# jkflying/opencalibration

Hardware: AMD Instinct MI355X
Metric: images/sec end-to-end (extract+match+relax) on synthetic aerial grid; LM iters/sec (higher is better)
Workload: dtype f32 (extract) + fp4 0/1 bits, f32 accumulate, exact (match) + f64 (RANSAC, relax)

## Files before the change

include/oc_host.h:

```cpp
#ifndef OC_HOST_H
#define OC_HOST_H

#include <stddef.h>
#include <stdint.h>

#include "ochip.h"

#ifdef __cplusplus
extern "C"
{
#endif

    size_t och_subsample(const double *loc, const float *strength, size_t n, double spacing, size_t count,
                         uint64_t *out);

    size_t och_matches_from_device(const ochip_match *raw, const uint64_t *idx1, size_t n1, const uint64_t *idx2,
                                   size_t n2, uint64_t *out_i1, uint64_t *out_i2, double *out_dist);

    typedef struct och_graph och_graph;
    och_graph *och_graph_create(void);
    void och_graph_destroy(och_graph *g);
    const char *och_last_error(const och_graph *g);
    uint32_t och_graph_add_model(och_graph *g, const double *m10);
    uint64_t och_graph_add_image(och_graph *g, const double *loc, const float *strength, const uint64_t *desc, size_t n,
                                 size_t num_sparse, uint32_t model, const double *position3);
    uint64_t och_graph_add_edge(och_graph *g, uint64_t source_id, uint64_t dest_id, const double *H9, int is_homography,
                                size_t n_inliers, const double *inl_px4, const uint64_t *inl_idx3, size_t n_matches,
                                const uint64_t *match_idx2, const double *match_dist, const double *poses32);
    void och_graph_get_orientations(const och_graph *g, double *ori );
    void och_link_match_work(const och_graph *g, double *out3);
    size_t och_graph_num_nodes(const och_graph *g);
    size_t och_graph_num_edges(const och_graph *g);
    void och_graph_node_ids(const och_graph *g, uint64_t *out);
    int och_link_stage_run(och_graph *g, ochip_ctx *ctx, const uint64_t *node_ids, size_t n, int keep_debug,
                           double *timers);
    size_t och_link_debug_count(const och_graph *g);
    void och_link_debug_pair(const och_graph *g, size_t p, uint64_t *ids2, uint64_t *n_matches, double *score,
                             uint32_t *iters3);
    void och_link_debug_matches(const och_graph *g, size_t p, uint64_t *i1, uint64_t *i2, double *dist, uint8_t *inl);
    void och_graph_edge_info(const och_graph *g, size_t e, uint64_t *ids2, uint64_t *counts2, double *H, double *poses);
    void och_graph_edge_inliers(const och_graph *g, size_t e, uint64_t *f1, uint64_t *f2, uint64_t *match_index,
                                double *px4);
    void och_graph_edge_match_distances(const och_graph *g, size_t e, double *out);
    void och_graph_edge_matches(const och_graph *g, size_t e, uint64_t *idx2, double *dist, int *is_homography);
    void och_graph_set_orientations(och_graph *g, const double *ori );

    int och_extract_features_batch(ochip_ctx *ctx, const uint8_t *images_bgr, uint32_t n_images, int width, int height,
                                   uint32_t max_keypoints, uint32_t max_out, double *loc, float *strength,
                                   uint64_t *desc, uint32_t *counts, uint32_t *num_sparse, int images_on_device);
    const char *och_extract_last_error(void);
    int och_homography_decompose(const double *H9, const double *m1m2, size_t n, double *poses);
    void och_image_to_3d(const double *px, size_t n, const double *model10, double *rays);
    double och_ransac_epipolar(ochip_ctx *ctx, int model, const double *rays6, const double *quality, size_t n, double threshold,
                               double *M9, uint8_t *inliers, uint32_t *counts3);
    size_t och_extract_tail(const float *kp6, const uint64_t *desc, uint32_t n, double scale, double *loc, float *strength,
                            uint64_t *desc_out, uint64_t *num_sparse);
    size_t och_extract_tail_prepared(const uint8_t *records, const float *response, const uint32_t *slot, uint32_t num_sparse_in,
                                     int conflict, uint32_t n, double scale, double *loc, float *strength, uint64_t *desc_out,
                                     uint64_t *num_sparse);
    void och_extract_tail_profile(double *out5);
    void och_sort_by_response(const float *response, uint32_t n, uint32_t *order_out, int use_std);
    int och_graph_load_images(och_graph *g, ochip_ctx *ctx, const uint8_t *images_bgr, uint32_t n_images, int width,
                              int height, uint32_t max_keypoints, int images_on_device, uint32_t model,
                              const double *positions, uint64_t *node_ids_out, double *totals2);

    int och_graph_load_link_images(och_graph *g, ochip_ctx *ctx, const uint8_t *images_bgr, uint32_t n_images, int width,
                                   int height, uint32_t max_keypoints, int images_on_device, uint32_t model,
                                   const double *positions, const double *orientations, uint64_t *node_ids_out,
                                   double *totals2, double *link_timers8, double *stage_seconds2);

    typedef struct och_initial_processing och_initial_processing;
    och_initial_processing *och_initial_processing_create(och_graph *g, ochip_ctx *ctx);
    void och_initial_processing_destroy(och_initial_processing *ip);
    int och_initial_processing_pending(const och_initial_processing *ip);
    int och_initial_processing_step(och_initial_processing *ip, const uint8_t *images_bgr, uint32_t n_images, int width, int height,
                                    uint32_t max_keypoints, int images_on_device, uint32_t model, const double *positions,
                                    int sequential, uint64_t *node_ids_out, double *stats16);

    typedef struct och_shard och_shard;
    void och_shard_block(uint32_t n_images, uint32_t rank, uint32_t world, uint32_t *first, uint32_t *count);
    och_shard *och_shard_begin(och_graph *g, ochip_ctx *ctx, uint32_t n_images, uint32_t model, const double *positions,
                               const double *orientations, uint32_t rank, uint32_t world, uint64_t *node_ids_out);
    void och_shard_destroy(och_shard *s);
    void och_shard_counts(const och_shard *s, uint64_t *counts4);
    int och_shard_load_link_local(och_shard *s, const uint8_t *images_bgr, int width, int height, uint32_t max_keypoints,
                                  int images_on_device);
    int och_shard_subsets_export(och_shard *s, const void **buf, uint64_t *bytes);
    int och_shard_subsets_import(och_shard *s, const void *buf, uint64_t bytes);
    int och_shard_link_remote(och_shard *s);
    int och_shard_edges_export(och_shard *s, const void **buf, uint64_t *bytes);
    int och_shard_edges_import(och_shard *s, const void *buf, uint64_t bytes);
    int och_shard_finalize(och_shard *s, double *totals2, double *link_timers8, double *seconds9);

    int och_relax_ground_plane(ochip_ctx *ctx, size_t n_nodes, const double *node_pos, const double *node_ori,
                               const double *model10, size_t n_poses, const uint64_t *pose_node, double *pose_ori,
                               size_t n_edges, const uint64_t *edge_src, const uint64_t *edge_dst,
                               const double *edge_H, const uint8_t *edge_is_homography, const uint64_t *inl_off,
                               const double *inl_px, const uint64_t *inl_match_index, const uint64_t *dist_off,
                               const double *dist, size_t n_opt_edges, const uint64_t *opt_edges, double *plane_out,
                               double *summary_out);
    const char *och_relax_last_error(void);
    int och_debug_relax_setup_check(int on);
    int och_graph_relax_ground_plane(och_graph *g, ochip_ctx *ctx, double *ori_inout, double *plane_out,
                                     double *summary_out);
    int och_graph_relax_ground_plane_sharded(och_graph *g, ochip_ctx *ctx, double *ori_inout, double *plane_out,
                                             double *summary_out, uint32_t rank, uint32_t world,
                                             ochip_relax_exchange_fn exchange, void *user);

    typedef struct och_surface och_surface;
    och_surface *och_surface_create(void);
    void och_surface_destroy(och_surface *s);
    void och_surface_counts(const och_surface *s, size_t *n_vertices, size_t *n_edges, size_t *n_cloud);
    void och_surface_get(const och_surface *s, double *vertices, uint64_t *edges5, double *cloud);
    void och_surface_set(och_surface *s, size_t n_vertices, const double *vertices, size_t n_edges, const uint64_t *edges5,
                         size_t n_cloud, const double *cloud);
    void och_surface_set_heights(och_surface *s, const double *z);
    void och_rebuild_mesh(const double *cam_xyz, size_t n, const och_surface *previous, int minimal, och_surface *out);
    int och_relax(ochip_ctx *ctx, size_t n_nodes, const double *node_pos, const double *node_ori, const double *model10,
                  const uint64_t *feat_off, const double *feat_xy, size_t n_poses, const uint64_t *pose_node,
                  double *pose_ori, size_t n_edges, const uint64_t *edge_src, const uint64_t *edge_dst, const double *edge_H,
                  const uint8_t *edge_is_homography, const uint64_t *inl_off, const double *inl_px,
                  const uint64_t *inl_feat, const uint64_t *inl_match_index, const uint64_t *dist_off, const double *dist,
                  size_t n_opt_edges, const uint64_t *opt_edges, uint32_t options, double grid_fraction,
                  const och_surface *previous, och_surface *surface_out, double *summary_out, double *model10_inout);
    int och_relax_ex(ochip_ctx *ctx, size_t n_nodes, const double *node_pos, const double *node_ori, const double *model10,
                     const uint64_t *feat_off, const double *feat_xy, size_t n_poses, const uint64_t *pose_node,
                     double *pose_ori, size_t n_edges, const uint64_t *edge_src, const uint64_t *edge_dst, const double *edge_H,
                     const uint8_t *edge_is_homography, const uint64_t *inl_off, const double *inl_px,
                     const uint64_t *inl_feat, const uint64_t *inl_match_index, const uint64_t *dist_off, const double *dist,
                     size_t n_opt_edges, const uint64_t *opt_edges, uint32_t options, double grid_fraction,
                     const och_surface *previous, och_surface *surface_out, double *summary_out, double *model10_inout,
                     const double *edge_poses32, int points_mode, double *points_before, double *points_after,
                     size_t points_cap, size_t *n_points_out);
    int och_graph_relax(och_graph *g, ochip_ctx *ctx, double *ori_inout, uint32_t options, double grid_fraction,
                        const och_surface *previous, och_surface *surface_out, double *summary_out);

    int och_graph_relax_sharded(och_graph *g, ochip_ctx *ctx, double *ori_inout, uint32_t options, double grid_fraction,
                                const och_surface *previous, och_surface *surface_out, double *summary_out, uint32_t rank,
                                uint32_t world, ochip_relax_exchange_fn exchange, void *user);

    int och_relax_stage_run(och_graph *g, ochip_ctx *ctx, const uint64_t *node_ids, size_t n_ids, int relax_all,
                            int disable_parallelism, uint32_t options, double grid_fraction, size_t max_groups,
                            const och_surface *previous, och_surface *surface_out, int64_t *group_of_node,
                            double *summary_out);
    typedef struct och_relax_stage och_relax_stage;
    och_relax_stage *och_relax_stage_begin(och_graph *g, const uint64_t *node_ids, size_t n_ids, int relax_all,
                                           int disable_parallelism, uint32_t options, double grid_fraction, size_t max_groups,
                                           const och_surface *previous, int64_t *group_of_node);
    size_t och_relax_stage_num_groups(const och_relax_stage *st);
    int och_relax_stage_run_groups(och_relax_stage *st, ochip_ctx *ctx, uint32_t rank, uint32_t world);
    int och_relax_stage_export(och_relax_stage *st, uint32_t rank, uint32_t world, const void **buf, uint64_t *bytes);
    int och_relax_stage_import(och_relax_stage *st, const void *buf, uint64_t bytes);
    int och_relax_stage_end(och_relax_stage *st, och_surface *surface_out, double *summary_out);
    size_t och_relax_partition(const och_graph *g, size_t num_groups, int64_t *group_of_node, int64_t *position_in_group);
    void och_convert_model(const double *m10, int to_inverse, double *out10);
    void och_merge_surfaces(const och_surface *const *surfaces, size_t n, och_surface *out);

    int och_graph_set_model(och_graph *g, uint32_t model, const double *m10);
    int och_graph_refit_edges(och_graph *g, ochip_ctx *ctx);

    char *och_graph_to_json(const och_graph *g, size_t *len);
    void och_free(void *p);
    int och_graph_from_json(och_graph *g, const char *text, size_t len);
    int och_graph_save_json(och_graph *g, const char *path);
    int och_graph_load_json(och_graph *g, const char *path);
    void och_graph_node_table(const och_graph *g, uint64_t *ids, uint32_t *model_index, uint64_t *n_features, uint64_t *n_sparse);
    int och_graph_node_payload(const och_graph *g, size_t index, double *loc, float *strength, uint64_t *desc,
                               double *position3, double *orientation4);
    const char *och_graph_node_path(const och_graph *g, size_t index);
    int och_graph_set_node_path(och_graph *g, size_t index, const char *path);
    size_t och_graph_num_models(const och_graph *g);
    int och_graph_get_model(const och_graph *g, uint32_t index, double *m11);
    int och_surface_save_ply(const och_surface *s, const char *path);
    int och_surface_load_ply(och_surface *s, const char *path);
    size_t och_surface_num_clouds(const och_surface *s);
    void och_surface_cloud_sizes(const och_surface *s, uint64_t *sizes);
    void och_surface_set_clouds(och_surface *s, size_t n_clouds, const uint64_t *sizes, const double *xyz);
    typedef struct och_checkpoint och_checkpoint;
    int och_checkpoint_validate(const char *dir);
    int och_checkpoint_save(const char *dir, och_graph *g, const och_surface *const *surfaces, size_t n_surfaces,
                            const char *state, const double *info4);
    och_checkpoint *och_checkpoint_load(const char *dir, och_graph *g);
    void och_checkpoint_destroy(och_checkpoint *cp);
    size_t och_checkpoint_num_surfaces(const och_checkpoint *cp);
    const char *och_checkpoint_state(const och_checkpoint *cp);
    void och_checkpoint_info(const och_checkpoint *cp, double *info4);
    int och_checkpoint_get_surface(const och_checkpoint *cp, size_t index, och_surface *out);

    int och_densify_mesh(och_graph *g, ochip_ctx *ctx, och_surface *surface, double *stats10, uint64_t *match_pairs,
                         size_t match_cap);
    uint32_t och_hilbert_xy2d(int order, int x, int y);

    size_t och_refine_by_point_density(och_surface *s, size_t max_points_per_triangle, double min_distance_variance,
                                       int max_iterations, double min_triangle_size);
    size_t och_refine_at_point(och_surface *s, double x, double y, int levels);
    size_t och_count_points_per_triangle(const och_surface *s, uint64_t *tri3, double *stats2, size_t cap);
    void och_surface_locate(const och_surface *s, const double *xy, size_t n, uint64_t *tri3);
    int och_mesh_refinement_run(och_graph *g, ochip_ctx *ctx, och_surface *surface, int max_steps, double *log8);

    typedef struct och_point_counter och_point_counter;
    const char *och_points_last_error(void);
    size_t och_surface_count_points(const och_surface *s, ochip_ctx *ctx, uint64_t *tri3, double *stats2, size_t cap);
    int och_surface_locate_on(const och_surface *s, ochip_ctx *ctx, const double *xy, size_t n, int max_steps, uint64_t *tri3);
    och_point_counter *och_point_counter_create(ochip_ctx *ctx, const double *xyz, size_t n, int max_steps);
    void och_point_counter_destroy(och_point_counter *c);
    size_t och_point_counter_count(och_point_counter *c, const och_surface *s, uint64_t *tri3, double *stats2, size_t cap,
                                   uint64_t *exhausted);
    void och_surface_locate_table_sizes(const och_surface *s, uint64_t *sizes2);
    void och_surface_locate_table(const och_surface *s, double *vertex_xy, uint32_t *neighbours, double *plane, double *cx, double *cy,
                                  double *grid4, uint32_t *start, uint32_t *items);
    int och_dense_mesh_relax_run(och_graph *g, ochip_ctx *ctx, och_surface *surface, int max_steps, double *log6);

    int och_graph_set_thumbnail(och_graph *g, size_t node_index, size_t rows, size_t cols, const uint8_t *rgb );
    void och_ortho_bounds(const och_surface *const *surfaces, size_t n, double *bounds5);
    double och_ortho_gsd(const och_graph *g, const uint64_t *node_ids, size_t n_ids, double mean_surface_z, int thumbnail);
    size_t och_ortho_context(const och_graph *g, const och_surface *const *surfaces, size_t n, int thumbnail, double *ctx8);
    void och_ortho_clamp_resolution(uint64_t total_input_pixels, double *gsd, int32_t *width, int32_t *height);
    void och_ortho_clamp_megapixels(double max_output_megapixels, double *gsd, int32_t *width, int32_t *height);
    double och_ray_trace_height(const och_surface *const *surfaces, size_t n, double x, double y, double mean_camera_z);
    int och_orthomosaic_thumbnail(och_graph *g, ochip_ctx *ctx, const och_surface *const *surfaces, size_t n, const double *z_in,
                                  double *plan8, uint8_t *rgba, uint32_t *ids, double *z_out);
    int och_dsm_plan(const och_graph *g, const och_surface *const *surfaces, size_t n, double max_output_megapixels, double *plan8);
    int och_ortho_mesh_upload(ochip_ctx *ctx, const och_surface *const *surfaces, size_t n, ochip_ortho_mesh **out);
    int och_dsm_render(ochip_ctx *ctx, ochip_ortho_mesh *dev, const och_surface *const *surfaces, size_t n, const double *plan8,
                       int64_t row0, int64_t rows, float *out, int out_on_device, uint32_t *tri_out, double *z64_out,
                       uint64_t *capped_walks);
    const char *och_ortho_last_error(void);
    size_t och_ortho_layers_cameras(const och_graph *g, const och_surface *const *surfaces, size_t n, double *cams,
                                    uint64_t *node_ids, uint32_t *model_ids, int64_t *image_hw);
    int och_ortho_layers_render(const och_graph *g, ochip_ctx *ctx, ochip_ortho_mesh *dev, const och_surface *const *surfaces,
                                size_t n, const double *plan8, const int32_t *config4, int64_t row0, int64_t rows,
                                const uint64_t *images, const int64_t *image_hw, const float *dsm_in, int out_on_device,
                                uint8_t *bgra, uint64_t *ids, float *weight, ochip_color_corr *corr_out, uint64_t corr_capacity,
                                uint64_t *n_corr, uint32_t *knn_out);
    const char *och_ortho_layers_last_error(void);
    void och_lab_convert(int mode, const uint8_t *in, size_t n, void *out);
    int och_ortho_patch_sample(const double *cam28, const uint8_t *img, double gsd, const double *xyz, uint8_t *bgr_out,
                               double *pixel2, double *J4);
    void och_ortho_sample_fields(double pixel_x, double pixel_y, int32_t width, int32_t height, float camera_distance,
                                 double cos_view, float *out5);
    int och_ortho_band_cameras(ochip_ctx *ctx, const double *raster4, int32_t cols, int64_t rows, int64_t band_rows, size_t n_cams,
                               const double *cams, uint8_t *used);
    int och_ortho_layers_render_subset(const och_graph *g, ochip_ctx *ctx, ochip_ortho_mesh *dev, const och_surface *const *surfaces,
                                       size_t n, const double *plan8, const int32_t *config4, int64_t row0, int64_t rows,
                                       const uint32_t *subset, size_t n_subset, const uint64_t *images, const int64_t *image_hw,
                                       const float *dsm_in, int out_on_device, uint8_t *bgra, uint64_t *ids, float *weight,
                                       ochip_color_corr *corr_out, uint64_t corr_capacity, uint64_t *n_corr, uint32_t *knn_out);
    int och_ortho_residency_plan(const uint8_t *used, size_t n_bands, size_t n_cams, size_t capacity, int32_t *resident,
                                 size_t *load_off, int32_t *loads3);
    typedef struct och_ortho_stream och_ortho_stream;
    int och_ortho_stream_create(const och_graph *g, ochip_ctx *ctx, ochip_ortho_mesh *mesh, const och_surface *const *surfaces,
// ... 63 lines not shown
```

include/ochip.h:

```cpp
#ifndef OCHIP_H
#define OCHIP_H

#include <stddef.h>
#include <stdint.h>

#ifdef __cplusplus
extern "C"
{
#endif

#define OCHIP_OK 0
#define OCHIP_EINVAL (-1)
#define OCHIP_ENOMEM (-2)
#define OCHIP_EHIP (-3)
#define OCHIP_ENODEV (-4)
#define OCHIP_ESTATE (-5)

#define OCHIP_DESC_WORDS64 8
#define OCHIP_DESC_BITS 486
#define OCHIP_NO_SECOND 0xFFFFu

    typedef struct ochip_ctx ochip_ctx;

    typedef struct ochip_pair
    {
        uint32_t image_1;
        uint32_t image_2;
    } ochip_pair;

    typedef struct ochip_match
    {
        uint32_t best_k;
        uint16_t best_count;
        uint16_t second_count;
    } ochip_match;

    enum
    {
        OCHIP_K_MATCH = 0,
        OCHIP_K_RANSAC = 1,
        OCHIP_K_RELAX_EVAL = 2,
        OCHIP_K_RELAX_SOLVE = 3,
        OCHIP_K_AKAZE = 4,
        OCHIP_K_DENSE = 5,
        OCHIP_K_COUNT = 8
    };

    int ochip_ctx_create(int device, ochip_ctx **out);
    void ochip_ctx_destroy(ochip_ctx *ctx);
    int ochip_ctx_sibling(ochip_ctx *ctx, uint32_t index, ochip_ctx **out);
    uint64_t ochip_akaze_progress(const ochip_ctx *ctx);
    void *ochip_ctx_attachment(ochip_ctx *ctx, void *(*make)(void), void (*destroy)(void *));
    int ochip_ctx_set_priority(ochip_ctx *ctx, int high);
    const char *ochip_last_error(const ochip_ctx *ctx);
    int ochip_device_info(const ochip_ctx *ctx, char *name, size_t name_len, int *compute_units, size_t *hbm_bytes);
    int ochip_synchronize(ochip_ctx *ctx);

    int ochip_descriptors_reserve(ochip_ctx *ctx, uint32_t n_images, uint64_t total_descriptors);
    int ochip_upload_descriptors(ochip_ctx *ctx, uint32_t image_id, const uint64_t *desc, uint32_t n);
    int ochip_descriptor_count(const ochip_ctx *ctx, uint32_t image_id, uint32_t *n);

    int ochip_match_batch(ochip_ctx *ctx, const ochip_pair *pairs, uint32_t n_pairs, const uint64_t *out_offset,
                          ochip_match *out);
    int ochip_match_sort(ochip_ctx *ctx, const ochip_pair *pairs, uint32_t n_pairs, const uint64_t *out_offset, uint64_t out_total,
                         uint32_t *counts_out, uint8_t *fallback_out);
    int ochip_match_launch(ochip_ctx *ctx, const ochip_pair *pairs, uint32_t n_pairs, const uint64_t *out_offset,
                           uint64_t out_total);
    int ochip_match_fetch(ochip_ctx *ctx, ochip_match *out, uint64_t out_total);

    int ochip_akaze_batch(ochip_ctx *ctx, const uint8_t *images_bgr, uint32_t n_images, int width, int height,
                          uint32_t max_kp, float *kp6, uint64_t *desc, uint32_t *counts, int *work_wh);

    int ochip_akaze_batch_dev(ochip_ctx *ctx, const uint8_t *images_bgr_dev, uint32_t n_images, int width, int height,
                              uint32_t max_kp, float *kp6, uint64_t *desc, uint32_t *counts, int *work_wh);

#define OCHIP_SUBSET_CAP 16384
    typedef struct ochip_feature_lists
    {
        uint8_t *records;
        float *response;
        uint32_t *slot;
        uint32_t *num_sparse;
        uint8_t *conflict;
        uint32_t *subset;
        uint32_t *num_subset;
        uint8_t *subset_conflict;
        double subset_spacing;
    } ochip_feature_lists;
    int ochip_akaze_features(ochip_ctx *ctx, const uint8_t *images_bgr, uint32_t n_images, int width, int height, uint32_t max_kp,
                             double nms_radius, uint32_t *counts, const ochip_feature_lists *lists, int *work_wh);
    int ochip_akaze_features_dev(ochip_ctx *ctx, const uint8_t *images_bgr_dev, uint32_t n_images, int width, int height,
                                 uint32_t max_kp, double nms_radius, uint32_t *counts, const ochip_feature_lists *lists, int *work_wh);
    int ochip_feature_lists_from_keypoints(ochip_ctx *ctx, const float *kp6, const uint64_t *desc, const uint32_t *counts, uint32_t n_images,
                            uint32_t max_kp, int work_w, int work_h, double scale, double nms_radius,
                            const ochip_feature_lists *out);

    int ochip_synth_views_alloc(ochip_ctx *ctx, uint32_t n_images, int width, int height, uint8_t **images_dev);
    void ochip_synth_views_free(ochip_ctx *ctx, uint8_t *images_dev);
    int ochip_synth_views_read(ochip_ctx *ctx, const uint8_t *images_dev, uint32_t index, int width, int height,
                               uint8_t *host_out);
    int ochip_synth_render_views(ochip_ctx *ctx, uint8_t *images_dev, uint32_t first_image, uint32_t n_images, int width,
                                 int height, const double *cams, const double *model3, const double *plane2,
                                 const double *lattice3, uint32_t seed);

    int ochip_upload_keypoints(ochip_ctx *ctx, uint32_t image_id, const double *xy, uint32_t n, const double *model8);

    int ochip_upload_batch(ochip_ctx *ctx, uint32_t n_images, const uint32_t *counts, const uint64_t *desc_all,
                           const double *xy_all, const double *models8);

    int ochip_host_alloc(ochip_ctx *ctx, size_t bytes, void **out);
    void ochip_host_free(ochip_ctx *ctx, void *p);

    typedef struct ochip_ransac_match
    {
        uint32_t k1, k2;
        uint16_t count;
        uint16_t reserved;
    } ochip_ransac_match;

    typedef struct ochip_ransac_job
    {
        uint32_t image_1, image_2;
        uint32_t n;
        uint32_t rng_state;
        uint64_t match_offset;
        uint64_t eval_offset;
    } ochip_ransac_job;

    typedef struct ochip_ransac_result
    {
        double H[9];
        double score;
        uint32_t iterations;
        uint32_t n_inliers;
        uint32_t improvements;
        uint32_t reserved;
    } ochip_ransac_result;

    int ochip_ransac_homography_batch(ochip_ctx *ctx, const ochip_ransac_job *jobs, uint32_t n_jobs,
                                      const ochip_ransac_match *matches, const uint32_t *sorted_idx,
                                      uint64_t total_matches, const uint32_t *eval_order, uint64_t eval_total,
                                      double inlier_threshold, ochip_ransac_result *results, uint8_t *inliers);

    typedef struct ochip_epipolar_job
    {
        uint32_t n;
        uint32_t rng_state;
        uint32_t has_quality;
        uint32_t reserved;
        uint64_t corr_offset;
        uint64_t eval_offset;
    } ochip_epipolar_job;
    int ochip_ransac_epipolar_batch(ochip_ctx *ctx, int model, const ochip_epipolar_job *jobs, uint32_t n_jobs,
                                    const double *corr6, const uint32_t *sorted_idx, uint64_t total,
                                    const uint32_t *eval_order, uint64_t eval_total, double inlier_threshold,
                                    ochip_ransac_result *results, uint8_t *inliers);

    typedef struct ochip_decomposition
    {
        double pose[4][8];
        uint32_t can_decompose, n_inliers;
    } ochip_decomposition;
    int ochip_ransac_homography_batch_sorted(ochip_ctx *ctx, const ochip_ransac_job *jobs, uint32_t n_jobs, uint64_t total_matches,
                                             const uint32_t *eval_order, uint64_t eval_total, double inlier_threshold,
                                             ochip_ransac_result *results, uint8_t *inliers, ochip_ransac_match *matches_out,
                                             uint8_t *fallback_out, ochip_decomposition *decomp_out);
    int ochip_edge_lists(ochip_ctx *ctx, uint32_t n_jobs, uint64_t total_matches, const uint32_t *feature_index, uint64_t n_keypoints,
                         const uint64_t *inlier_offset, uint64_t total_inliers, void *feature_match_out, void *inlier_match_out);
    int ochip_refit_homography_batch(ochip_ctx *ctx, const ochip_ransac_job *jobs, uint32_t n_jobs,
                                     const ochip_ransac_match *matches, uint64_t total_matches, uint32_t rounds,
                                     double inlier_threshold, ochip_ransac_result *results, uint8_t *inliers);

    int ochip_debug_homography_fit4(ochip_ctx *ctx, int route, const double *xy16, uint32_t n, double *H9, double *Hinv9,
                                    uint8_t *degenerate);

// ... 349 lines not shown
```

opencalibration_amd/capi.py:

```python
import ctypes as C
import os

import numpy as np

_HERE = os.path.dirname(os.path.abspath(__file__))
LIB_PATH = os.path.join(_HERE, "libochip.so")

K_MATCH, K_RANSAC, K_RELAX_EVAL, K_RELAX_SOLVE, K_AKAZE = 0, 1, 2, 3, 4
NO_SECOND = 0xFFFF

PAIR_DTYPE = np.dtype([("image_1", np.uint32), ("image_2", np.uint32)])
MATCH_DTYPE = np.dtype([("best_k", np.uint32), ("best_count", np.uint16), ("second_count", np.uint16)])
RANSAC_JOB_DTYPE = np.dtype([("image_1", np.uint32), ("image_2", np.uint32), ("n", np.uint32), ("rng_state", np.uint32),
                             ("match_offset", np.uint64), ("eval_offset", np.uint64)])
RANSAC_MATCH_DTYPE = np.dtype([("k1", np.uint32), ("k2", np.uint32), ("count", np.uint16), ("reserved", np.uint16)])
RANSAC_RESULT_DTYPE = np.dtype([("H", np.float64, (9,)), ("score", np.float64), ("iterations", np.uint32), ("n_inliers", np.uint32),
                                ("improvements", np.uint32), ("reserved", np.uint32)])

EXPORTS = [
    "ochip_ctx_create", "ochip_ctx_destroy", "ochip_ctx_sibling", "ochip_ctx_attachment", "ochip_akaze_progress", "ochip_ctx_set_priority", "ochip_last_error", "ochip_device_info", "ochip_synchronize",
    "ochip_descriptors_reserve", "ochip_upload_descriptors", "ochip_descriptor_count",
    "ochip_match_batch", "ochip_match_launch", "ochip_match_fetch",
    "ochip_upload_keypoints", "ochip_ransac_homography_batch", "ochip_refit_homography_batch", "ochip_ransac_epipolar_batch",
    "ochip_upload_batch", "ochip_host_alloc", "ochip_host_free", "ochip_akaze_batch", "ochip_akaze_batch_dev", "ochip_akaze_features", "ochip_akaze_features_dev", "ochip_feature_lists_from_keypoints",
    "ochip_synth_views_alloc", "ochip_synth_views_free", "ochip_synth_render_views", "ochip_synth_views_read",
    "ochip_relax_problem_create", "ochip_relax_problem_destroy", "ochip_relax_set_cameras_constant",
    "ochip_relax_solve", "ochip_relax_get_state", "ochip_relax_set_shard", "ochip_relax_evaluate",
    "ochip_plane_setup_create", "ochip_plane_setup_override", "ochip_plane_setup_blocks", "ochip_plane_setup_destroy",
    "ochip_plane_chain_create", "ochip_plane_chain_run", "ochip_plane_chain_destroy",
    "ochip_relaxg_problem_create", "ochip_relaxg_problem_destroy", "ochip_relaxg_set_structure_only", "ochip_relaxg_solve",
    "ochip_relaxg_get_state", "ochip_relaxg_evaluate", "ochip_relaxg_set_exchange",
    "ochip_relaxp_problem_create", "ochip_relaxp_problem_destroy", "ochip_relaxp_set_structure_only", "ochip_relaxp_solve",
    "ochip_relaxp_get_state", "ochip_relaxp_evaluate", "ochip_relaxp_step",
    "ochip_profile_reset", "ochip_profile_get", "ochip_match_work", "ochip_relax_work", "ochip_relax_memory", "ochip_work_counters",
    "ochip_debug_fp64", "ochip_debug_std_sort", "ochip_debug_lm_step", "ochip_debug_homography_fit4", "ochip_match_sort", "ochip_ransac_homography_batch_sorted", "ochip_edge_lists",
    "ochip_dense_index_create", "ochip_dense_index_destroy", "ochip_dense_match", "ochip_dense_link", "ochip_dense_triangulate",
    "ochip_rccl_unique_id", "ochip_rccl_comm_create", "ochip_rccl_comm_destroy", "ochip_rccl_comm_stats",
    "ochip_rccl_relax_exchange",
    "ochip_ortho_mesh_create", "ochip_ortho_mesh_destroy", "ochip_ortho_dsm", "ochip_ortho_thumbnail", "ochip_ortho_layers",
    "ochip_ortho_blend", "ochip_laplacian_blend",
    "ochip_ortho_band_cameras", "ochip_image_slots_create", "ochip_image_slots_destroy", "ochip_image_slots_address",
    "ochip_image_slots_upload", "ochip_image_slots_mark", "ochip_image_slots_wait", "ochip_image_slots_elapsed",
    "ochip_color_balance_solve", "ochip_color_balance_evaluate",
    "ochip_thumbnail_size", "ochip_image_thumbnails", "ochip_debug_lab_table",
    "ochip_ortho_overviews_levels", "ochip_ortho_overviews_create", "ochip_ortho_overviews_feed",
    "ochip_ortho_overviews_complete_rows", "ochip_ortho_overviews_finish", "ochip_ortho_overviews_destroy",
    "ochip_mesh_points_create", "ochip_mesh_points_size", "ochip_mesh_points_count", "ochip_mesh_points_where",
    "ochip_mesh_points_destroy",
]

_lib = None


class RelaxDesc(C.Structure):
    _fields_ = [("n_cams", C.c_uint32), ("cam_pos", C.c_void_p), ("cam_q", C.c_void_p), ("cam_optimize", C.c_void_p),
                ("plane_xy", C.c_double * 6), ("plane_z", C.c_double * 3), ("z_optimize", C.c_uint8 * 3),
                ("n_blocks", C.c_uint32), ("blk_cam_a", C.c_void_p), ("blk_cam_b", C.c_void_p), ("blk_rays", C.c_void_p),
                ("n_prior", C.c_uint32), ("prior_cam", C.c_void_p), ("huber_a", C.c_double), ("prior_weight", C.c_double)]


class RelaxOptions(C.Structure):
    _fields_ = [("max_num_iterations", C.c_int), ("initial_trust_region_radius", C.c_double),
                ("function_tolerance", C.c_double), ("gradient_tolerance", C.c_double), ("parameter_tolerance", C.c_double)]


class RelaxSummary(C.Structure):
    _fields_ = [("termination", C.c_int), ("iterations", C.c_int), ("successful_steps", C.c_int),
                ("unsuccessful_steps", C.c_int), ("num_parameters", C.c_int), ("num_residual_blocks", C.c_int),
                ("initial_cost", C.c_double), ("final_cost", C.c_double)]


def relax_desc(scene):
    d = RelaxDesc()
    keep = []

    def arr(name, dtype):
        a = np.ascontiguousarray(scene[name], dtype).reshape(-1)
        a = a if a.size else np.zeros(1, dtype)
        keep.append(a)
        return a.ctypes.data

    d.n_cams = len(scene["cam_pos"])
    d.cam_pos, d.cam_q, d.cam_optimize = arr("cam_pos", np.float64), arr("cam_q", np.float64), arr("cam_optimize", np.uint8)
    for i in range(6):
        d.plane_xy[i] = float(np.reshape(scene["plane_xy"], -1)[i])
    for i in range(3):
        d.plane_z[i] = float(scene["plane_z"][i])
        d.z_optimize[i] = int(scene["z_optimize"][i])
    d.n_blocks = len(scene["blk_cam_a"])
    d.blk_cam_a, d.blk_cam_b = arr("blk_cam_a", np.uint32), arr("blk_cam_b", np.uint32)
    d.blk_rays = arr("blk_rays", np.float64)
    d.n_prior, d.prior_cam = len(scene["prior_cam"]), arr("prior_cam", np.uint32)
    d.huber_a, d.prior_weight = scene["huber_a"], scene["prior_weight"]
    return d, keep


class RelaxgDesc(C.Structure):
    _fields_ = [("n_cams", C.c_uint32), ("cam_pos", C.c_void_p), ("cam_q", C.c_void_p), ("cam_optimize", C.c_void_p),
                ("n_verts", C.c_uint32), ("vert_xy", C.c_void_p), ("vert_z", C.c_void_p), ("vert_optimize", C.c_void_p),
                ("n_blocks", C.c_uint32), ("blk_n", C.c_void_p), ("blk_intr", C.c_void_p), ("blk_ray_off", C.c_void_p),
                ("blk_tri", C.c_void_p), ("ray_cam", C.c_void_p), ("ray_dir", C.c_void_p), ("ray_px", C.c_void_p),
                ("n_down", C.c_uint32), ("down_cam", C.c_void_p), ("down_weight", C.c_double),
                ("n_diff", C.c_uint32), ("diff_v", C.c_void_p), ("diff_weight", C.c_double), ("anchor_weight", C.c_double),
                ("n_smooth", C.c_uint32), ("smooth_v", C.c_void_p), ("smooth_weight", C.c_double), ("huber_a", C.c_double),
                ("model", C.c_double * 8), ("opt_focal", C.c_uint8), ("opt_principal", C.c_uint8), ("n_radial_free", C.c_uint8),
                ("focal_lo", C.c_double), ("focal_hi", C.c_double), ("mono_observations", C.c_uint32), ("mono_r_max", C.c_double),
                ("shard_rank", C.c_uint32), ("shard_world", C.c_uint32),
# ... 641 lines not shown
```

opencalibration_amd/csrc/akaze.hip:

```cpp
#include "area_table.hpp"
#include "ctx.hpp"

#include <algorithm>
#include <cmath>
#include <limits>
#include <cstring>
#include <type_traits>
#include <vector>

namespace
{

struct level_info
{
    int octave, w, h, sigma_size;
    float esigma;
    size_t off;
    int tile_off, tiles_x;
    int mask_off;
    int sup_off, sup_tx;
};

__device__ __forceinline__ int clampi(int v, int lo, int hi)
{
// ... 2502 lines not shown
    if (n <= 0)
        return tau;
    const double scale = 3.0 * t / (tau_max * (double)(n * (n + 1)));
    const double c = 1.0 / (4.0 * n + 2.0), d = scale * tau_max / 2.0;
    std::vector<double> tauh(n);
    for (int k = 0; k < n; k++)
    {
        const double hh = std::cos(M_PI * (2.0 * k + 1.0) * c);
        tauh[k] = d / (hh * hh);
    }
    tau.resize(n);
    const int kappa = n / 2;
    int prime = n + 1;
    while (!is_prime(prime))
        prime++;
    for (int k = 0, l = 0; l < n; ++k, ++l)
    {
        int index = 0;
        while ((index = ((k + 1) * kappa) % prime - 1) >= n)
            k++;
        tau[l] = (float)tauh[index];
    }
    return tau;
}

__device__ __forceinline__ uint32_t hash32(uint32_t x)
{
    x ^= x >> 16;
    x *= 0x7feb352dU;
    x ^= x >> 15;
    x *= 0x846ca68bU;
    x ^= x >> 16;
    return x;
}
__device__ __forceinline__ float hashf(uint32_t x)
{
    return (float)(hash32(x) >> 8) * (1.0f / 16777216.0f);
}
struct synth_cam
{
    float pos[3], q[4];
};
__global__ void render_views_kernel(uint8_t *__restrict__ out, int w, int h, const synth_cam *__restrict__ cams, float f,
                                    float ppx, float ppy, float pa, float pb, float x0, float y0, float spacing,
                                    uint32_t seed)
{
    const int x = blockIdx.x * blockDim.x + threadIdx.x, y = blockIdx.y;
    if (x >= w)
        return;
    const synth_cam c = cams[blockIdx.z];
    const float ux = ((float)x - ppx) / f, uy = ((float)y - ppy) / f;
    const float qx = c.q[0], qy = c.q[1], qz = c.q[2], qw = c.q[3];
    float uvx = qy * 1.0f - qz * uy, uvy = qz * ux - qx * 1.0f, uvz = qx * uy - qy * ux;
    uvx += uvx;
    uvy += uvy;
    uvz += uvz;
    const float dx = ux + qw * uvx + (qy * uvz - qz * uvy), dy = uy + qw * uvy + (qz * uvx - qx * uvz),
                dz = 1.0f + qw * uvz + (qx * uvy - qy * uvx);
    const float t = (pa * c.pos[0] + pb * c.pos[1] - c.pos[2]) / (dz - pa * dx - pb * dy);
    const float gx = c.pos[0] + t * dx, gy = c.pos[1] + t * dy;
    const int ci = (int)floorf((gx - x0) / spacing), cj = (int)floorf((gy - y0) / spacing);
    float v = 0.5f;
    for (int di = -1; di <= 1; di++)
        for (int dj = -1; dj <= 1; dj++)
        {
            const uint32_t id = (uint32_t)(ci + di) * 73856093u ^ (uint32_t)(cj + dj) * 19349663u ^ seed;
            const float bx = x0 + ((float)(ci + di) + 0.5f + 0.6f * (hashf(id) - 0.5f)) * spacing;
            const float by = y0 + ((float)(cj + dj) + 0.5f + 0.6f * (hashf(id + 1) - 0.5f)) * spacing;
            const float amp = (0.25f + 0.5f * hashf(id + 2)) * ((hash32(id + 3) & 1) ? 1.0f : -1.0f);
            const float sg = spacing * (0.10f + 0.14f * hashf(id + 4));
            const float r2 = (gx - bx) * (gx - bx) + (gy - by) * (gy - by);
            v += amp * __expf(-r2 / (2.0f * sg * sg));
        }
    const float o = fminf(255.0f, fmaxf(0.0f, v * 255.0f));
    const uint8_t g = (uint8_t)o;
    uint8_t *p = out + ((size_t)blockIdx.z * w * h + (size_t)y * w + x) * 3;
    p[0] = g;
    p[1] = g;
    p[2] = g;
}

int akaze_run(ochip_ctx *ctx, const uint8_t *images_bgr, bool on_device, uint32_t n_images, int width, int height,
              uint32_t max_kp, float *kp6, uint64_t *desc, uint32_t *counts, int *work_wh,
              const ochip_feature_lists *lists = nullptr, double nms_radius = 8.0);

}

extern "C"
{

int ochip_akaze_batch(ochip_ctx *ctx, const uint8_t *images_bgr, uint32_t n_images, int width, int height,
                      uint32_t max_kp, float *kp6, uint64_t *desc, uint32_t *counts, int *work_wh)
{
    return akaze_run(ctx, images_bgr, false, n_images, width, height, max_kp, kp6, desc, counts, work_wh);
}

int ochip_akaze_batch_dev(ochip_ctx *ctx, const uint8_t *images_bgr_dev, uint32_t n_images, int width, int height,
                          uint32_t max_kp, float *kp6, uint64_t *desc, uint32_t *counts, int *work_wh)
{
    return akaze_run(ctx, images_bgr_dev, true, n_images, width, height, max_kp, kp6, desc, counts, work_wh);
}

int ochip_akaze_features(ochip_ctx *ctx, const uint8_t *images_bgr, uint32_t n_images, int width, int height, uint32_t max_kp,
                         double nms_radius, uint32_t *counts, const ochip_feature_lists *lists, int *work_wh)
{
    if (!lists || !lists->records || !lists->response || !lists->slot || !lists->num_sparse || !lists->conflict)
        return OCHIP_EINVAL;
    return akaze_run(ctx, images_bgr, false, n_images, width, height, max_kp, nullptr, nullptr, counts, work_wh, lists, nms_radius);
}

int ochip_akaze_features_dev(ochip_ctx *ctx, const uint8_t *images_bgr_dev, uint32_t n_images, int width, int height, uint32_t max_kp,
                             double nms_radius, uint32_t *counts, const ochip_feature_lists *lists, int *work_wh)
{
    if (!lists || !lists->records || !lists->response || !lists->slot || !lists->num_sparse || !lists->conflict)
        return OCHIP_EINVAL;
    return akaze_run(ctx, images_bgr_dev, true, n_images, width, height, max_kp, nullptr, nullptr, counts, work_wh, lists, nms_radius);
}

int ochip_synth_views_alloc(ochip_ctx *ctx, uint32_t n_images, int width, int height, uint8_t **images_dev)
{
    if (!ctx || !images_dev)
        return OCHIP_EINVAL;
    OCHIP_HIP(ctx, hipSetDevice(ctx->device));
    *images_dev = nullptr;
    if (hipMalloc((void **)images_dev, (size_t)(n_images ? n_images : 1) * width * height * 3) != hipSuccess)
        return ochip_fail(ctx, OCHIP_ENOMEM, "hipMalloc(%zu) for synthetic views failed", (size_t)n_images * width * height * 3);
    return OCHIP_OK;
}

int ochip_synth_views_read(ochip_ctx *ctx, const uint8_t *images_dev, uint32_t index, int width, int height,
                           uint8_t *host_out)
{
    if (!ctx || !images_dev || !host_out)
        return OCHIP_EINVAL;
    OCHIP_HIP(ctx, hipSetDevice(ctx->device));
    const size_t bytes = (size_t)width * height * 3;
    OCHIP_HIP(ctx, hipMemcpy(host_out, images_dev + (size_t)index * bytes, bytes, hipMemcpyDeviceToHost));
    return OCHIP_OK;
}

void ochip_synth_views_free(ochip_ctx *ctx, uint8_t *images_dev)
{
    if (ctx && images_dev)
    {
        (void)hipSetDevice(ctx->device);
        (void)hipFree(images_dev);
    }
}

int ochip_synth_render_views(ochip_ctx *ctx, uint8_t *images_dev, uint32_t first_image, uint32_t n_images, int width,
                             int height, const double *cams, const double *model3, const double *plane2,
                             const double *lattice3, uint32_t seed)
{
    if (!ctx || !images_dev || !cams || !model3 || !plane2 || !lattice3)
        return OCHIP_EINVAL;
    if (n_images == 0)
        return OCHIP_OK;
    OCHIP_HIP(ctx, hipSetDevice(ctx->device));
    std::vector<synth_cam> hc(n_images);
    for (uint32_t i = 0; i < n_images; i++)
    {
        for (int k = 0; k < 3; k++)
            hc[i].pos[k] = (float)cams[7 * i + k];
        for (int k = 0; k < 4; k++)
            hc[i].q[k] = (float)cams[7 * i + 3 + k];
    }
    synth_cam *dc = nullptr;
    if (hipMalloc((void **)&dc, n_images * sizeof(synth_cam)) != hipSuccess)
        return ochip_fail(ctx, OCHIP_ENOMEM, "hipMalloc failed");
    hipError_t e = hipMemcpy(dc, hc.data(), n_images * sizeof(synth_cam), hipMemcpyHostToDevice);
    if (e == hipSuccess)
    {
        hipLaunchKernelGGL(render_views_kernel, dim3((width + 255) / 256, height, n_images), dim3(256), 0, ctx->stream,
                           images_dev + (size_t)first_image * width * height * 3, width, height, (const synth_cam *)dc,
                           (float)model3[0], (float)model3[1], (float)model3[2], (float)plane2[0], (float)plane2[1],
                           (float)lattice3[0], (float)lattice3[1], (float)lattice3[2], seed);
        e = ochip_stream_wait(ctx, ctx->stream);
    }
    (void)hipFree(dc);
    if (e != hipSuccess)
        return ochip_fail(ctx, OCHIP_EHIP, "ochip_synth_render_views: %s", hipGetErrorString(e));
    return OCHIP_OK;
}

}

struct ochip::akaze_tables
{
    ochip::dev_blocks mem;
    int width = 0, height = 0, W = 0, H = 0, n_levels = 0, n_tiles = 0;
    unsigned int *tile_seq = nullptr;
    void *gtab = nullptr;
    int *xo = nullptr, *xs = nullptr, *yo = nullptr, *ys = nullptr;
    float *xa = nullptr, *ya = nullptr;
    bool staged = false;
    int most_taps = 0;
};

namespace
// ... 111 lines not shown
        ctx->akaze_tabs->mem.ctx = ctx;
        ctx->akaze_tabs->mem.what = "akaze tables";
        ctx->akaze_tabs_destroy = [](ochip::akaze_tables *t) {
            t->mem.release();
            delete t;
        };
    }
    ochip::akaze_tables &T = *ctx->akaze_tabs;
    *out = &T;
    if (T.width == width && T.height == height && T.W == W && T.H == H && T.n_levels == LV.n && T.n_tiles == n_tiles)
        return OCHIP_OK;
    T.width = 0;
    T.mem.release();
    constexpr auto ENQ = ochip::copy_mode::enqueue;
    int rc = OCHIP_OK;
    std::vector<std::pair<uint64_t, unsigned int>> keyed;
    keyed.reserve(n_tiles);
    auto spread = [](uint32_t v) {
        uint64_t x = v;
        x = (x | (x << 16)) & 0x0000FFFF0000FFFFull;
        x = (x | (x << 8)) & 0x00FF00FF00FF00FFull;
        x = (x | (x << 4)) & 0x0F0F0F0F0F0F0F0Full;
        x = (x | (x << 2)) & 0x3333333333333333ull;
        x = (x | (x << 1)) & 0x5555555555555555ull;
        return x;
    };
    for (int i = 0; i < LV.n; i++)
    {
        const level_info &l = LV.l[i];
        const int ty_n = (l.h + DT_Y - 1) / DT_Y;
        for (int ty = 0; ty < ty_n; ty++)
            for (int tx = 0; tx < l.tiles_x; tx++)
                keyed.emplace_back(((uint64_t)i << 48) | spread((uint32_t)tx) | (spread((uint32_t)ty) << 1),
                                   (unsigned int)(l.tile_off + ty * l.tiles_x + tx));
    }
    std::sort(keyed.begin(), keyed.end());
    std::vector<unsigned int> seq(keyed.size());
    for (size_t i = 0; i < keyed.size(); i++)
        seq[i] = keyed[i].second;
    rc = rc != OCHIP_OK ? rc : T.mem.upload(&T.tile_seq, seq, ENQ);
    gather_tab *g = nullptr;
    rc = rc != OCHIP_OK ? rc : T.mem.upload(&g, &host_gather_tab(), 1, ENQ);
    T.gtab = g;
    area_tab tx, ty;
    T.staged = false;
    T.most_taps = 0;
    if (!(W == width && H == height))
    {
        tx = area_table(width, W, 1.0 / scale);
        ty = area_table(height, H, 1.0 / scale);
        bool staged = width % 4 == 0;
        for (int x0 = 0; x0 < W && staged; x0 += 256)
        {
            const int x1 = std::min(x0 + 256, W);
            const int c0 = tx.si[tx.off[x0]] & ~3, c1 = tx.si[tx.off[x1] - 1];
            staged = c1 - c0 + 1 <= RS_PITCH - 3;
            for (int x = x0; x < x1 && staged; x++)
                staged = tx.off[x + 1] - tx.off[x] <= RESIZE_MAX_TAPS;
        }
        for (int y0 = 0; y0 < H && staged; y0 += RESIZE_ROWS)
        {
            const int y1 = std::min(y0 + RESIZE_ROWS, H);
            staged = ty.si[ty.off[y1] - 1] - ty.si[ty.off[y0]] + 1 <= RS_ROWS;
        }
        T.staged = staged;
        for (int x = 0; x < W; x++)
            T.most_taps = std::max(T.most_taps, tx.off[x + 1] - tx.off[x]);
        rc = rc != OCHIP_OK ? rc : T.mem.upload(&T.xo, tx.off, ENQ);
        rc = rc != OCHIP_OK ? rc : T.mem.upload(&T.xs, tx.si, ENQ);
        rc = rc != OCHIP_OK ? rc : T.mem.upload(&T.xa, tx.alpha, ENQ);
        rc = rc != OCHIP_OK ? rc : T.mem.upload(&T.yo, ty.off, ENQ);
        rc = rc != OCHIP_OK ? rc : T.mem.upload(&T.ys, ty.si, ENQ);
        rc = rc != OCHIP_OK ? rc : T.mem.upload(&T.ya, ty.alpha, ENQ);
    }
    OCHIP_HIP(ctx, ochip_stream_wait(ctx, ctx->stream));
    if (rc != OCHIP_OK)
        return rc;
    T.width = width, T.height = height, T.W = W, T.H = H, T.n_levels = LV.n, T.n_tiles = n_tiles;
    return OCHIP_OK;
}

int akaze_run(ochip_ctx *ctx, const uint8_t *images_bgr, bool on_device, uint32_t n_images, int width, int height,
              uint32_t max_kp, float *kp6, uint64_t *desc, uint32_t *counts, int *work_wh, const ochip_feature_lists *lists,
              double nms_radius)
{
    if (!ctx || !counts || (n_images && (!images_bgr || (!lists && (!kp6 || !desc)))))
        return OCHIP_EINVAL;
    if (width <= 0 || height <= 0)
        return ochip_fail(ctx, OCHIP_EINVAL, "bad image size %d x %d", width, height);
    OCHIP_HIP(ctx, hipSetDevice(ctx->device));
    hipStream_t st = ctx->stream;
    const double scale = std::min(1.f, float(1600) / (float)std::max(width, height));
    const int W = (int)std::lrint(width * scale), H = (int)std::lrint(height * scale);
    if (work_wh)
    {
        work_wh[0] = W;
        work_wh[1] = H;
    }
    for (uint32_t i = 0; i < n_images; i++)
        counts[i] = 0;
    if (n_images == 0)
        return OCHIP_OK;

    const int omax = 4, nsub = 4;
    const float soffset = 1.6f, dfactor = 1.5f, dthreshold = 0.00005f;
    levels_dev LV{};
    std::vector<std::vector<float>> tsteps;
    size_t img_stride = 0;
    int n_tiles = 0;
    size_t mask_stride = 0;
    size_t sup_stride = 0;
    {
        std::vector<float> etime;
        for (int i = 0; i < omax; i++)
        {
            const float rfactor = 1.0f / (float)(1 << i);
            const int lw = (int)(W * rfactor), lh = (int)(H * rfactor);
            if ((lw < 80 || lh < 40) && i != 0)
                break;
            for (int j = 0; j < nsub; j++)
            {
                level_info &l = LV.l[LV.n++];
                l.octave = i;
                l.w = lw;
                l.h = lh;
                l.esigma = soffset * std::pow(2.0f, (float)j / (float)nsub + (float)i);
                l.sigma_size = (int)std::lrintf(l.esigma * dfactor / (float)(1 << i));
                l.off = img_stride;
                img_stride += (size_t)lw * lh;
                l.tiles_x = (lw + BT_X - 1) / BT_X;
                l.tile_off = n_tiles;
                n_tiles += l.tiles_x * ((lh + DT_Y - 1) / DT_Y);
                l.mask_off = (int)mask_stride;
                mask_stride += (size_t)l.tiles_x * lh;
                l.sup_off = (int)sup_stride;
                l.sup_tx = (lw + 7) / 8;
                sup_stride += (size_t)l.sup_tx * ((lh + 7) / 8);
                etime.push_back(0.5f * (l.esigma * l.esigma));
            }
        }
        tsteps.resize(LV.n);
        for (int i = 1; i < LV.n; i++)
            tsteps[i] = fed_taus(etime[i] - etime[i - 1], 0.25f);
    }
    const size_t plane0 = (size_t)W * H;
    const uint32_t B = n_images;
    const uint32_t max_cands = std::max<uint32_t>(max_kp * 4, 1u << 16);

    ochip::dev_scratch mem{ctx, "akaze"};
    constexpr auto WAIT = ochip::copy_mode::enqueue_wait;
    int rc = OCHIP_OK;
#define AK(call)                                                                                                       \
    do                                                                                                                 \
    {                                                                                                                  \
        if (rc == OCHIP_OK)                                                                                            \
            rc = (call);                                                                                               \
    } while (0)
    uint8_t *d_bgr = nullptr, *d_gray = nullptr;
    float *d_img = nullptr, *d_flow = nullptr, *d_ping = nullptr;
    float2 *d_Lxy = nullptr;
    float2 *d_Fit = nullptr;
    float *d_Lt = nullptr, *d_Rmax = nullptr, *d_kc = nullptr,
          *d_kp = nullptr;
    unsigned int *d_hmax = nullptr, *d_hist = nullptr, *d_ncand = nullptr, *d_pmax = nullptr;
    cand_t *d_cands = nullptr;
    unsigned char *d_dead = nullptr, *d_valid = nullptr;
    unsigned long long *d_desc = nullptr, *d_descc = nullptr;
// ... 444 lines not shown
        OCHIP_HIP(ctx, hipMemsetAsync(d_waiting, 0, (size_t)B * LV.n * 4, st));
        hipLaunchKernelGGL(suppress_level_first_kernel, dim3(B), dim3(64), 0, st, (const unsigned int *)d_ncand, max_cands, LV,
                           (const unsigned int *)d_tile_base, (const unsigned int *)d_tile_seq, n_tiles, d_level_first);
        hipLaunchKernelGGL(suppress_tiles_kernel, dim3((unsigned int)((LV.l[0].tiles_x * ((LV.l[0].h + 7) / 8) + 255) / 256), LV.n, B),
                           dim3(256), 0, st, (const unsigned long long *)d_mask, mask_stride, d_rmask, sup_stride, LV);
#define SUP_PASS(PASS, LEVELS)                                                                                                                 \
    hipLaunchKernelGGL(suppress_round0_kernel<PASS>, per_cand, dim3(256), 0, st, (const cand_t *)d_cands, (const unsigned int *)d_ncand,       \
                       max_cands, (const float *)d_Rmax, img_stride, (const unsigned long long *)d_rmask, d_pmask, d_kmask, sup_stride, LV,    \
                       (const unsigned int *)d_level_first, d_turns, d_waiting, (const unsigned int *)d_found, sup_hooks);                     \
    hipLaunchKernelGGL(suppress_rounds_kernel<PASS>, dim3(B, (LEVELS)), dim3(SUP_THREADS), 0, st, (const unsigned int *)d_ncand, max_cands,    \
                       (const float *)d_Rmax, img_stride, d_pmask, d_kmask, sup_stride, LV, (const unsigned int *)d_level_first, d_turns,      \
                       d_waiting, d_sup_stats, sup_hooks)
#define SUP_WINDOWS(PASS)                                                                                                                      \
    OCHIP_HIP(ctx, hipMemsetAsync(d_rmask, 0, (size_t)B * sup_stride * 8, st));                                                                \
    hipLaunchKernelGGL(suppress_window_kernel<PASS>, per_cand, dim3(256), 0, st, (const cand_t *)d_cands, (const unsigned int *)d_ncand,       \
                       max_cands, (const unsigned long long *)d_kmask, d_rmask, sup_stride, LV, d_found, sup_hooks)
        SUP_PASS(1, LV.n);
        if (LV.n > 1)
        {
            SUP_WINDOWS(2);
            SUP_PASS(2, LV.n - 1);
            SUP_WINDOWS(3);
            SUP_PASS(3, LV.n - 1);
        }
#undef SUP_WINDOWS
        hipLaunchKernelGGL(suppress_dead_kernel, per_cand, dim3(256), 0, st, (const cand_t *)d_cands, (const unsigned int *)d_ncand,
                           max_cands, (const unsigned long long *)d_kmask, sup_stride, LV, d_dead);
        if (d_sup_stats)
        {
            std::vector<unsigned int> hs((size_t)3 * B * LV.n * 3);
            OCHIP_HIP(ctx, hipMemcpyAsync(hs.data(), d_sup_stats, hs.size() * 4, hipMemcpyDeviceToHost, st));
            OCHIP_HIP(ctx, ochip_stream_wait(ctx, st));
            for (int pass = 0; pass < 3; pass++)
            {
                std::string line;
                for (int i = 0; i < LV.n; i++)
                {
                    unsigned int rounds = 0, ticks = 0, pts = 0;
                    for (uint32_t b = 0; b < B; b++)
                    {
                        const unsigned int *o = &hs[(((size_t)pass * B + b) * LV.n + i) * 3];
                        rounds = std::max(rounds, o[0]), ticks = std::max(ticks, o[1]), pts = std::max(pts, o[2]);
                    }
                    char buf[64];
                    std::snprintf(buf, sizeof buf, " %u/%.0fus/%u", rounds, ticks * 0.01, pts);
                    line += buf;
                }
                std::fprintf(stderr, "[ochip extract] suppression pass %d, per level max over %u images of rounds/time/points:%s\n", pass + 1, B,
                             line.c_str());
            }
        }
        hipLaunchKernelGGL(live_list_kernel, dim3(B), dim3(SCAN_THREADS), 0, st, (const unsigned char *)d_dead, (const unsigned int *)d_ncand,
                           max_cands, d_live, d_nlive);
        OCHIP_HIP(ctx, hipMemsetAsync(d_valid, 0, (size_t)B * max_cands, st));
        std::vector<unsigned int> nlive(B);
        OCHIP_HIP(ctx, hipMemcpyAsync(nlive.data(), d_nlive, B * 4, hipMemcpyDeviceToHost, st));
        OCHIP_HIP(ctx, ochip_stream_wait(ctx, st));
        const unsigned int max_live = *std::max_element(nlive.begin(), nlive.end());
        if (max_live > 0)
        {
            hipLaunchKernelGGL(describe3_kernel, dim3(512 * (((max_live + DESC_WPB - 1) / DESC_WPB + 511) / 512), 1, B), dim3(64 * DESC_WPB), 0, st,
                               (const cand_t *)d_cands, (const unsigned int *)d_nlive, max_cands, (const unsigned int *)d_live,
                               (const float *)d_Lt, (const float2 *)d_Lxy, img_stride, LV, dfactor,
                               (const gather_tab *)d_gtab, d_kp, d_desc, d_valid, xcd_remap, d_vmask,
                               mask_stride);
        }
    }
    if (max_n > 0)
    {
        hipLaunchKernelGGL(rank_scan_kernel, dim3(B), dim3(SCAN_THREADS), 0, st, (const unsigned long long *)d_vmask, mask_stride, d_wbase,
                           d_counts);
        hipLaunchKernelGGL(compact_ordered_kernel, dim3((max_n + 255) / 256, 1, B), dim3(256), 0, st,
                           (const unsigned char *)d_valid, (const cand_t *)d_cands, (const unsigned int *)d_ncand, max_cands,
                           (const unsigned long long *)d_vmask, (const unsigned int *)d_wbase, mask_stride, LV,
                           (const float *)d_kp, (const unsigned long long *)d_desc, d_kpc, d_descc, max_kp);
    }
    else
        OCHIP_HIP(ctx, hipMemsetAsync(d_counts, 0, B * 4, st));
    ochip_prof_end(ctx, OCHIP_K_AKAZE, e0, e1);
    OCHIP_HIP(ctx, hipGetLastError());
    OCHIP_HIP(ctx, hipMemcpyAsync(counts, d_counts, B * 4, hipMemcpyDeviceToHost, st));
    OCHIP_HIP(ctx, ochip_stream_wait(ctx, st));
    uint32_t most = 0;
    for (uint32_t b = 0; b < B && rc == OCHIP_OK; b++)
    {
        if (counts[b] > max_kp)
        {
            rc = ochip_fail(ctx, OCHIP_ENOMEM, "image %u has %u keypoints, more than max_kp = %u", b, counts[b], max_kp);
            break;
        }
        most = std::max(most, counts[b]);
    }
    if (rc == OCHIP_OK && lists)
        rc = ochip::feature_lists_enqueue(ctx, mem, B, max_kp, d_kpc, d_descc, d_counts, most, W, H, scale, nms_radius, lists);
    else if (rc == OCHIP_OK && most > 0)
    {
        OCHIP_HIP(ctx, hipMemcpy2DAsync(kp6, (size_t)max_kp * 24, d_kpc, (size_t)max_kp * 24, (size_t)most * 24, B, hipMemcpyDeviceToHost, st));
        OCHIP_HIP(ctx, hipMemcpy2DAsync(desc, (size_t)max_kp * 64, d_descc, (size_t)max_kp * 64, (size_t)most * 64, B, hipMemcpyDeviceToHost, st));
    }
    if (rc != OCHIP_OK)
        for (uint32_t b = 0; b < B; b++)
            counts[b] = 0;
    (void)ochip_stream_wait(ctx, st);
    mem.release();
    return rc;
#undef AK
}

}
```

opencalibration_amd/csrc/ctx.hip:

```cpp
#include "ctx.hpp"

#include <cstring>

static std::string g_create_error;

int ochip_fail(ochip_ctx *ctx, int code, const char *fmt, ...)
{
    char buf[512];
    va_list ap;
    va_start(ap, fmt);
    vsnprintf(buf, sizeof buf, fmt, ap);
    va_end(ap);
    if (ctx)
        ctx->error = buf;
    else
        g_create_error = buf;
    return code;
}

int ochip::dev_array_mem::grow(ochip_ctx *ctx, size_t want)
{
    if (mem)
        OCHIP_HIP(ctx, hipFree(mem));
    mem = nullptr;
// ... 189 lines not shown
    (void)hipEventRecord(stop, ctx->stream);
    auto &s = ctx->prof[kid];
    s.pending.emplace_back(start, stop);
    if (s.pending.size() >= 4096)
        prof_drain(ctx, kid);
}

extern "C"
{

int ochip_ctx_create(int device, ochip_ctx **out)
{
    if (!out)
        return ochip_fail(nullptr, OCHIP_EINVAL, "out is NULL");
    *out = nullptr;
    int count = 0;
    if (hipGetDeviceCount(&count) != hipSuccess || count <= 0)
        return ochip_fail(nullptr, OCHIP_ENODEV, "no HIP device visible");
    if (device < 0 || device >= count)
        return ochip_fail(nullptr, OCHIP_EINVAL, "device %d out of range (0..%d)", device, count - 1);
    ochip_ctx *ctx = new (std::nothrow) ochip_ctx();
    if (!ctx)
        return ochip_fail(nullptr, OCHIP_ENOMEM, "host allocation failed");
    ctx->device = ctx->stream.device = device;
    hipError_t e = hipSetDevice(device);
    const char *bsync = getenv("OCHIP_BLOCKING_SYNC");
    ctx->blocking_wait = !(bsync && bsync[0] == '0');
    if (e == hipSuccess && ctx->blocking_wait)
    {
        (void)hipSetDeviceFlags(hipDeviceScheduleBlockingSync);
        (void)hipGetLastError();
    }
    if (e == hipSuccess)
        e = hipGetDeviceProperties(&ctx->prop, device);
    if (e == hipSuccess && std::strncmp(ctx->prop.gcnArchName, "gfx950", 6) != 0)
    {
        int rc = ochip_fail(nullptr, OCHIP_ENODEV, "device %d is %s; libochip is built for gfx950 only", device,
                            ctx->prop.gcnArchName);
        delete ctx;
        return rc;
    }
    if (e != hipSuccess)
    {
        int rc = ochip_fail(nullptr, OCHIP_EHIP, "context creation failed: %s", hipGetErrorString(e));
        delete ctx;
        return rc;
    }
    *out = ctx;
    return OCHIP_OK;
}

void ochip_ctx_destroy(ochip_ctx *ctx)
{
    if (!ctx)
        return;
    if (ctx->attachment && ctx->attachment_destroy)
        ctx->attachment_destroy(ctx->attachment);
    ctx->attachment = nullptr;
    for (ochip_ctx *sib : ctx->siblings)
        ochip_ctx_destroy(sib);
    ctx->siblings.clear();
    (void)hipSetDevice(ctx->device);
    (void)hipDeviceSynchronize();
    for (auto &s : ctx->prof)
    {
        for (auto &p : s.pending)
            s.free_list.push_back(p);
        for (auto &p : s.free_list)
        {
            (void)hipEventDestroy(p.first);
            (void)hipEventDestroy(p.second);
        }
    }
    for (ochip::dev_array_mem *a : ctx->dev_arrays)
        a->release();
    if (ctx->akaze_tabs && ctx->akaze_tabs_destroy)
        ctx->akaze_tabs_destroy(ctx->akaze_tabs);
    ctx->akaze_tabs = nullptr;
    if (ctx->lab_table_mem)
    {
        ctx->lab_table_mem->release();
        delete ctx->lab_table_mem;
    }
    for (auto &b : ctx->dev_pool)
        (void)hipFree(b.first);
    for (auto &b : ctx->pinned_pool)
        (void)hipHostFree(b.first);
    for (auto &b : ctx->pinned_live)
        (void)hipHostFree(b.first);
    if (ctx->sync_event)
        (void)hipEventDestroy(ctx->sync_event);
    for (hipStream_t r : ctx->retired_streams)
        (void)hipStreamDestroy(r);
    if (ctx->stream.opened())
        (void)hipStreamDestroy(ctx->stream.s);
    if (ctx->copy_stream)
        (void)hipStreamDestroy(ctx->copy_stream);
    delete ctx;
}

int ochip_ctx_set_priority(ochip_ctx *ctx, int high)
{
    if (!ctx)
        return OCHIP_EINVAL;
    if (ctx->stream_priority == (high ? 1 : 0))
        return OCHIP_OK;
    if (!ctx->stream.opened())
    {
        ctx->stream.priority = ctx->stream_priority = high ? 1 : 0;
        return OCHIP_OK;
    }
    OCHIP_HIP(ctx, hipSetDevice(ctx->device));
    int least = 0, greatest = 0;
    OCHIP_HIP(ctx, hipDeviceGetStreamPriorityRange(&least, &greatest));
    OCHIP_HIP(ctx, hipStreamSynchronize(ctx->stream));
    hipStream_t s = nullptr;
    OCHIP_HIP(ctx, hipStreamCreateWithPriority(&s, hipStreamNonBlocking, high ? greatest : least));
    ctx->retired_streams.push_back(ctx->stream.s);
    ctx->stream.s = s;
    ctx->stream.priority = ctx->stream_priority = high ? 1 : 0;
    return OCHIP_OK;
}

int ochip_ctx_sibling(ochip_ctx *ctx, uint32_t index, ochip_ctx **out)
{
    if (!ctx || !out)
        return OCHIP_EINVAL;
    *out = nullptr;
    std::lock_guard<std::mutex> lock(ctx->siblings_mutex);
    if (index > 64)
        return ochip_fail(ctx, OCHIP_EINVAL, "sibling index %u out of range", index);
    while (ctx->siblings.size() <= index)
    {
        ochip_ctx *s = nullptr;
        const int rc = ochip_ctx_create(ctx->device, &s);
        if (rc != OCHIP_OK)
            return ochip_fail(ctx, rc, "sibling context: %s", ochip_last_error(nullptr));
        ctx->siblings.push_back(s);
    }
    *out = ctx->siblings[index];
    return OCHIP_OK;
}

void *ochip_ctx_attachment(ochip_ctx *ctx, void *(*make)(void), void (*destroy)(void *))
{
    if (!ctx)
        return nullptr;
    std::lock_guard<std::mutex> lock(ctx->siblings_mutex);
    if (!ctx->attachment && make)
    {
        ctx->attachment = make();
        ctx->attachment_destroy = destroy;
    }
    return ctx->attachment;
}

uint64_t ochip_akaze_progress(const ochip_ctx *ctx)
{
    return ctx ? ctx->akaze_readbacks.load(std::memory_order_acquire) : 0;
}

const char *ochip_last_error(const ochip_ctx *ctx)
{
    return ctx ? ctx->error.c_str() : g_create_error.c_str();
}

// ... 289 lines not shown
```

opencalibration_amd/csrc/ctx.hpp:

```cpp
#pragma once

#include <hip/hip_runtime.h>

#include <atomic>
#include <cstdarg>
#include <cstdio>
#include <mutex>
#include <string>
#include <vector>

#include "../../include/ochip.h"
#include "env.hpp"

struct ochip_profile_slot
{
    std::vector<std::pair<hipEvent_t, hipEvent_t>> pending;
    std::vector<std::pair<hipEvent_t, hipEvent_t>> free_list;
    uint64_t launches = 0;
    double total_ms = 0;
};

namespace ochip
{
struct dev_blocks;
// ... 87 lines not shown
    {
        ochip_ransac_result *results;
        uint8_t *inliers;
    };
    outputs outputs_of(uint32_t n_jobs) const
    {
        ochip_ransac_result *r = out.as<ochip_ransac_result>();
        return {r, reinterpret_cast<uint8_t *>(r + n_jobs)};
    }
    int ensure(ochip_ctx *ctx, ransac_writer who, uint32_t n_jobs, size_t job_bytes, uint64_t T, size_t corr_bytes, uint64_t eval_total,
               unsigned flags_per_corr);
};
}

struct ochip_ctx
{
    int device = 0;
    ochip_lazy_stream stream;
    hipStream_t copy_stream = nullptr;
    std::vector<hipStream_t> retired_streams;
    int stream_priority = -1;
    hipEvent_t sync_event = nullptr;
    bool blocking_wait = true;
    std::string error;
    hipDeviceProp_t prop{};

    ochip::dev_array<uint32_t> desc_dev;
    uint64_t desc_capacity = 0, desc_used = 0;
    uint32_t n_images = 0;
    std::vector<uint64_t> img_off;
    std::vector<uint32_t> img_n;
    std::vector<uint8_t> img_set;
    ochip::dev_array<uint64_t> img_off_dev;
    ochip::dev_array<uint32_t> img_n_dev;
    bool img_tables_dirty = true;

    ochip::dev_array<double> kp_xy_dev, rays_dev;
    ochip::dev_array<uint32_t> kp_image_dev;
    ochip::dev_array<double> models_dev;
    std::vector<uint8_t> kp_set;
    bool rays_dirty = false;
    bool kp_store_ready = false;

    ochip::dev_array<ochip_pair> pairs_dev;
    ochip::dev_array<uint64_t> out_off_dev;
    ochip::dev_array<ochip_match> match_out_dev;
    uint64_t match_out_total = 0;
    ochip::dev_array<unsigned long long> ms_recs_dev;
    ochip::dev_array<unsigned char> ms_seg_dev, ms_flag_dev;
    uint32_t ms_pairs = 0;
    ochip::dev_array<unsigned char> sym_jobs_dev;
    ochip::dev_array<uint2> sym_part_dev;
    ochip::dev_array<uint4> desc_fp4_dev;
    ochip::dev_array<float> desc_negpop_dev;
    ochip::dev_array<uint32_t> desc_pop_dev;
    uint64_t fp4_valid = 0;

    ochip::ransac_scratch ransac;

    std::vector<ochip::dev_array_mem *> dev_arrays;

    std::vector<std::pair<void *, size_t>> pinned_live, pinned_pool;
    std::vector<std::pair<void *, size_t>> dev_pool;

    ochip_profile_slot prof[OCHIP_K_COUNT];
    uint64_t match_computed = 0, match_delivered = 0;
    double relax_mfma_flops = 0;
    uint64_t ransac_hyp_corr = 0, relax_blocks_jac = 0, relax_blocks_cost = 0;
    uint64_t relax_system_bytes = 0, relax_system_dense_bytes = 0, relax_system_unknowns = 0;

    std::vector<ochip_ctx *> siblings;
    std::mutex siblings_mutex;

    std::atomic<uint64_t> akaze_readbacks{0};

    ochip::dev_blocks *lab_table_mem = nullptr;
    uint32_t *lab_table_dev = nullptr;
    void *lab_tables_dev = nullptr;
    float lab_table_fill_ms = 0;

    ochip::akaze_tables *akaze_tabs = nullptr;
    void (*akaze_tabs_destroy)(ochip::akaze_tables *) = nullptr;

    void *attachment = nullptr;
    void (*attachment_destroy)(void *) = nullptr;
};


inline hipError_t ochip_stream_wait(ochip_ctx *ctx, hipStream_t st)
{
    if (ctx->stream.error != hipSuccess)
        return ctx->stream.error;
    if (!ctx->blocking_wait)
        return hipStreamSynchronize(st);
    if (!ctx->sync_event)
    {
        const hipError_t e = hipEventCreateWithFlags(&ctx->sync_event, hipEventBlockingSync | hipEventDisableTiming);
        if (e != hipSuccess)
            return e;
    }
    const hipError_t e = hipEventRecord(ctx->sync_event, st);
    return e != hipSuccess ? e : hipEventSynchronize(ctx->sync_event);
}

inline hipError_t ochip_copy_stream(ochip_ctx *ctx, hipStream_t *out)
{
    hipError_t e = hipSuccess;
    if (!ctx->copy_stream)
        e = hipStreamCreateWithFlags(&ctx->copy_stream, hipStreamNonBlocking);
    *out = ctx->copy_stream;
    return e;
}

int ochip_fail(ochip_ctx *ctx, int code, const char *fmt, ...);
int ochip_ensure_keypoint_store(ochip_ctx *ctx, size_t n_keypoints, size_t n_images);
int ochip_upload_image_tables(ochip_ctx *ctx);
void *ochip_pool_get(ochip_ctx *ctx, size_t bytes, size_t *got);
void ochip_pool_put(ochip_ctx *ctx, void *p, size_t bytes);
void ochip_prof_begin(ochip_ctx *ctx, int kid, hipEvent_t *start, hipEvent_t *stop);
void ochip_prof_end(ochip_ctx *ctx, int kid, hipEvent_t start, hipEvent_t stop);

#define OCHIP_HIP(ctx, call)                                                                                           \
    do                                                                                                                 \
    {                                                                                                                  \
        hipError_t e__ = (call);                                                                                       \
        if (e__ != hipSuccess)                                                                                         \
            return ochip_fail((ctx), OCHIP_EHIP, "%s failed: %s (%s:%d)", #call, hipGetErrorString(e__), __FILE__,    \
                              __LINE__);                                                                               \
    } while (0)

#define OCHIP_TRY(call)                                                                                                \
    do                                                                                                                 \
    {                                                                                                                  \
        const int rc__ = (call);                                                                                       \
        if (rc__ != OCHIP_OK)                                                                                          \
            return rc__;                                                                                               \
    } while (0)

namespace ochip
{
enum class copy_mode
{
    enqueue,
    enqueue_wait,
    blocking
};

struct dev_blocks
{
    ochip_ctx *ctx = nullptr;
    const char *what = "";
    std::vector<std::pair<void *, size_t>> held;

    dev_blocks() = default;
    dev_blocks(ochip_ctx *c, const char *w) : ctx(c), what(w) {}
    dev_blocks(const dev_blocks &) = delete;
    dev_blocks &operator=(const dev_blocks &) = delete;

    void *get(size_t bytes);
    int upload_bytes(void **dst, const void *src, size_t bytes, copy_mode m);
    template <class T> int upload(T **dst, const T *src, size_t n, copy_mode m)
    {
        void *d = nullptr;
        const int rc = upload_bytes(&d, src, n * sizeof(T), m);
        if (rc == OCHIP_OK)
            *dst = (T *)d;
        return rc;
    }
    template <class T> int upload(T **dst, const std::vector<T> &v, copy_mode m)
    {
        return upload(dst, v.data(), v.size(), m);
    }
    template <class T> int alloc(T **dst, size_t n)
    {
        return upload<T>(dst, nullptr, n, copy_mode::enqueue);
    }
    void release();
    bool empty() const
    {
        return held.empty();
    }
};

struct dev_scratch : dev_blocks
{
    using dev_blocks::dev_blocks;
    ~dev_scratch();
};

int feature_lists_enqueue(ochip_ctx *ctx, dev_blocks &mem, uint32_t B, uint32_t max_kp, const float *d_kp6,
                          const unsigned long long *d_desc, const unsigned int *d_counts, uint32_t most, int work_w, int work_h,
                          double scale, double nms_radius, const ochip_feature_lists *out);

int std_sort_enqueue(ochip_ctx *ctx, dev_blocks &mem, unsigned long long *recs, size_t total_len, const unsigned int *seg_begin,
                     const unsigned int *seg_end, uint32_t n_segs, uint32_t max_len, unsigned char *fallback);
}
```

opencalibration_amd/csrc/features.hip:

```cpp
#include "ctx.hpp"

#include <algorithm>
#include <cstdlib>
#include <cstring>
#include <vector>

using namespace ochip;

namespace
{

enum : unsigned char
{
    UNDECIDED = 0,
    SPARSE = 1,
    DENSE = 2
};

struct nms_dev
{
    unsigned int B, S;
    const unsigned int *n;
    const double2 *loc;
    double cell, scale2, radius2;
// ... 240 lines not shown
    __syncthreads();
    if (t == 0)
        (SUBSET ? F.n_subset : F.n_sparse)[b] = n ? total_kept : 0u;
}

__global__ void feat_records_kernel(feat_dev F)
{
    const unsigned int b = blockIdx.z, r = blockIdx.x * blockDim.x + threadIdx.x;
    const unsigned int n = F.n[b];
    if (r == 0)
    {
        F.sub_begin[b] = b * F.S;
        F.sub_end[b] = b * F.S + (n ? F.n_sparse[b] : 0u);
    }
    if (r >= n)
        return;
    const size_t o = (size_t)b * F.S + r;
    const unsigned long long sorted = F.recs[o];
    const unsigned int s = (unsigned int)sorted;
    const size_t src = (size_t)b * F.max_kp + s;
    unsigned long long rec[11];
    const double2 l = F.loc[o];
    rec[0] = (unsigned long long)__double_as_longlong(l.x);
    rec[1] = (unsigned long long)__double_as_longlong(l.y);
    rec[2] = (unsigned long long)__float_as_uint(F.kp6[src * 6 + 4]);
#pragma unroll
    for (int w = 0; w < 8; w++)
        rec[3 + w] = F.desc[src * 8 + w];
    const unsigned int at = F.slot_of_rank[o];
    const unsigned int ns = F.n_sparse[b];
    unsigned long long *out = reinterpret_cast<unsigned long long *>(F.records + ((size_t)b * (F.S + 1) + at) * 88);
#pragma unroll
    for (int w = 0; w < 11; w++)
        out[w] = rec[w];
    if (r == 0)
    {
        unsigned long long *again = reinterpret_cast<unsigned long long *>(F.records + ((size_t)b * (F.S + 1) + ns) * 88);
#pragma unroll
        for (int w = 0; w < 11; w++)
            again[w] = rec[w];
    }
    F.slot[(size_t)b * F.S + s] = at;
    if (at < ns)
        F.sub_recs[(size_t)b * F.S + at] = (sorted & 0xFFFFFFFF00000000ull) | at;
}

__global__ __launch_bounds__(256) void feat_subset_ties_kernel(feat_dev F)
{
    const unsigned int b = blockIdx.x;
    const unsigned int n = F.n[b] ? F.n_sparse[b] : 0u;
    __shared__ int tied;
    if (threadIdx.x == 0)
        tied = 0;
    __syncthreads();
    const unsigned long long *r = F.sub_recs + (size_t)b * F.S;
    int mine = 0;
    for (unsigned int i = threadIdx.x; i + 1 < n; i += 256)
        mine |= (r[i] >> 32) == (r[i + 1] >> 32);
    if (mine)
        tied = 1;
    __syncthreads();
    if (threadIdx.x == 0 && !tied)
        F.sub_end[b] = F.sub_begin[b];
}

__global__ void feat_subset_loc_kernel(feat_dev F)
{
    const unsigned int b = blockIdx.z, r = blockIdx.x * blockDim.x + threadIdx.x;
    if (r >= F.n_sparse[b] || F.n[b] == 0)
        return;
    const size_t o = (size_t)b * F.S + r;
    const unsigned int at = (unsigned int)F.sub_recs[o];
    const double *rec = reinterpret_cast<const double *>(F.records + ((size_t)b * (F.S + 1) + at) * 88);
    F.sub_loc[o] = make_double2(rec[0], rec[1]);
}

}

namespace ochip
{

int feature_lists_enqueue(ochip_ctx *ctx, dev_blocks &mem, uint32_t B, uint32_t max_kp, const float *d_kp6,
                          const unsigned long long *d_desc, const unsigned int *d_counts, uint32_t most, int work_w, int work_h,
                          double scale, double nms_radius, const ochip_feature_lists *out)
{
    hipStream_t st = ctx->stream;
    if (B == 0)
        return OCHIP_OK;
    if (most == 0)
    {
        std::memset(out->conflict, 0, B);
        std::memset(out->num_sparse, 0, (size_t)B * 4);
        if (out->num_subset)
            std::memset(out->num_subset, 0, (size_t)B * 4);
        if (out->subset_conflict)
            std::memset(out->subset_conflict, 0, B);
        return OCHIP_OK;
    }
    if (most > 60000)
        return ochip_fail(ctx, OCHIP_EINVAL, "feature lists: %u keypoints in one image exceed the suppression kernel's 60 000", most);
    const bool want_subset = out->subset && out->num_subset && out->subset_conflict && out->subset_spacing > 0;
    feat_dev F{};
    F.B = B;
    F.S = (most + 63) / 64 * 64;
    F.max_kp = max_kp;
    F.kp6 = d_kp6;
    F.desc = d_desc;
    F.counts = d_counts;
    F.scale = scale;
    const size_t N = (size_t)B * F.S;
    auto dev = [&](size_t bytes) { return mem.get(bytes); };
    bool alloc_ok = true;
    auto make_nms = [&](const unsigned int *n, const double2 *loc, double radius_in_loc_units, double scale2, double radius2) {
        nms_dev M{};
        M.B = B;
        M.S = F.S;
        M.n = n;
        M.loc = loc;
        M.cell = radius_in_loc_units * 1.0625;
        M.scale2 = scale2;
        M.radius2 = radius2;
        M.gw = (int)((double)work_w / scale / M.cell) + 2;
        M.gh = (int)((double)work_h / scale / M.cell) + 2;
        const size_t n_cells = (size_t)M.gw * M.gh;
        M.cell_id = (unsigned int *)dev(N * 4);
        M.cell_start = (unsigned int *)dev((size_t)B * (n_cells + 1) * 4);
        M.cell_fill = (unsigned int *)dev((size_t)B * n_cells * 4);
        M.items = (unsigned int *)dev(N * 4);
        M.item_loc = (double2 *)dev(N * 16);
        M.state = (unsigned char *)dev(N);
        alloc_ok = alloc_ok && M.cell_id && M.cell_start && M.cell_fill && M.items && M.item_loc && M.state;
        return M;
    };
    F.n = (unsigned int *)dev((size_t)B * 4);
    F.recs = (unsigned long long *)dev(N * 8);
    F.seg_begin = (unsigned int *)dev((size_t)B * 4);
    F.seg_end = (unsigned int *)dev((size_t)B * 4);
    F.resp = (float *)dev(N * 4);
    F.loc = (double2 *)dev(N * 16);
    F.slot_of_rank = (unsigned int *)dev(N * 4);
    F.slot = (unsigned int *)dev(N * 4);
    F.n_sparse = (unsigned int *)dev((size_t)B * 4);
    F.records = (unsigned char *)dev((size_t)B * (F.S + 1) * 88);
    F.sub_recs = (unsigned long long *)dev(N * 8);
    F.sub_begin = (unsigned int *)dev((size_t)B * 4);
    F.sub_end = (unsigned int *)dev((size_t)B * 4);
    F.sub_loc = (double2 *)dev(N * 16);
    F.subset = (unsigned int *)dev(N * 4);
    F.n_subset = (unsigned int *)dev((size_t)B * 4);
    unsigned char *conflict = (unsigned char *)dev(B), *conflict2 = (unsigned char *)dev(B);
    if (!F.n || !F.recs || !F.seg_begin || !F.seg_end || !F.resp || !F.loc || !F.slot_of_rank || !F.slot || !F.n_sparse || !F.records ||
        !F.sub_recs || !F.sub_begin || !F.sub_end || !F.sub_loc || !F.subset || !F.n_subset || !conflict || !conflict2)
        return OCHIP_ENOMEM;
    nms_dev M8 = make_nms(F.n, F.loc, nms_radius / scale, scale * scale, nms_radius * nms_radius);
    nms_dev M40{};
    if (want_subset)
        M40 = make_nms(F.n_sparse, F.sub_loc, out->subset_spacing, 1.0, out->subset_spacing * out->subset_spacing);
    if (!alloc_ok)
        return OCHIP_ENOMEM;
    const dim3 wide((F.S + 255) / 256, 1, B);
    constexpr int rounds = 6;
    auto suppress = [&](const nms_dev &M, bool subset) -> int {
        OCHIP_HIP(ctx, hipMemsetAsync(M.cell_fill, 0, (size_t)B * M.gw * M.gh * 4, st));
        hipLaunchKernelGGL(nms_cells_kernel, wide, dim3(256), 0, st, M);
        hipLaunchKernelGGL(nms_scan_kernel, dim3(B), dim3(SCAN_THREADS), 0, st, M);
        hipLaunchKernelGGL(nms_fill_kernel, wide, dim3(256), 0, st, M);
        for (int k = 0; k < rounds; k++)
            hipLaunchKernelGGL(nms_round_kernel, wide, dim3(256), 0, st, M);
        if (subset)
            hipLaunchKernelGGL(nms_finish_kernel<true>, dim3(B), dim3(FIN_THREADS), (size_t)F.S, st, M, F);
        else
            hipLaunchKernelGGL(nms_finish_kernel<false>, dim3(B), dim3(FIN_THREADS), (size_t)F.S, st, M, F);
        return OCHIP_OK;
    };
    hipLaunchKernelGGL(feat_keys_kernel, wide, dim3(256), 0, st, F);
    {
        const int src = std_sort_enqueue(ctx, mem, F.recs, N, F.seg_begin, F.seg_end, B, most, conflict);
        if (src != OCHIP_OK)
            return src;
    }
    hipLaunchKernelGGL(feat_loc_kernel, wide, dim3(256), 0, st, F);
    {
        const int rc = suppress(M8, false);
        if (rc != OCHIP_OK)
            return rc;
    }
    hipLaunchKernelGGL(feat_records_kernel, wide, dim3(256), 0, st, F);
    if (want_subset)
    {
        hipLaunchKernelGGL(feat_subset_ties_kernel, dim3(B), dim3(256), 0, st, F);
        const int src = std_sort_enqueue(ctx, mem, F.sub_recs, N, F.sub_begin, F.sub_end, B, most, conflict2);
        if (src != OCHIP_OK)
            return src;
        hipLaunchKernelGGL(feat_subset_loc_kernel, wide, dim3(256), 0, st, F);
        const int rc = suppress(M40, true);
        if (rc != OCHIP_OK)
            return rc;
    }
    OCHIP_HIP(ctx, hipGetLastError());
    OCHIP_HIP(ctx, hipMemcpy2DAsync(out->records, ((size_t)max_kp + 1) * 88, F.records, ((size_t)F.S + 1) * 88, ((size_t)most + 1) * 88, B,
                                    hipMemcpyDeviceToHost, st));
    OCHIP_HIP(ctx, hipMemcpy2DAsync(out->response, (size_t)max_kp * 4, F.resp, (size_t)F.S * 4, (size_t)most * 4, B, hipMemcpyDeviceToHost, st));
    OCHIP_HIP(ctx, hipMemcpy2DAsync(out->slot, (size_t)max_kp * 4, F.slot, (size_t)F.S * 4, (size_t)most * 4, B, hipMemcpyDeviceToHost, st));
    OCHIP_HIP(ctx, hipMemcpyAsync(out->num_sparse, F.n_sparse, (size_t)B * 4, hipMemcpyDeviceToHost, st));
    if (want_subset)
    {
        const size_t width = std::min<size_t>(most, OCHIP_SUBSET_CAP);
        OCHIP_HIP(ctx, hipMemcpy2DAsync(out->subset, (size_t)OCHIP_SUBSET_CAP * 4, F.subset, (size_t)F.S * 4, width * 4, B,
                                        hipMemcpyDeviceToHost, st));
        OCHIP_HIP(ctx, hipMemcpyAsync(out->num_subset, F.n_subset, (size_t)B * 4, hipMemcpyDeviceToHost, st));
        OCHIP_HIP(ctx, hipMemcpyAsync(out->subset_conflict, conflict2, B, hipMemcpyDeviceToHost, st));
    }
    OCHIP_HIP(ctx, hipMemcpyAsync(out->conflict, conflict, B, hipMemcpyDeviceToHost, st));
    return OCHIP_OK;
}

}

extern "C" int ochip_feature_lists_from_keypoints(ochip_ctx *ctx, const float *kp6, const uint64_t *desc, const uint32_t *counts,
                                                  uint32_t n_images, uint32_t max_kp, int work_w, int work_h, double scale,
                                                  double nms_radius, const ochip_feature_lists *out)
{
    if (!ctx || !out || !counts || (n_images && (!kp6 || !desc)) || !out->records || !out->response || !out->slot || !out->num_sparse ||
        !out->conflict)
        return OCHIP_EINVAL;
    OCHIP_HIP(ctx, hipSetDevice(ctx->device));
    hipStream_t st = ctx->stream;
    uint32_t most = 0;
    for (uint32_t b = 0; b < n_images; b++)
    {
        if (counts[b] > max_kp)
            return ochip_fail(ctx, OCHIP_EINVAL, "image %u: %u keypoints, more than max_kp = %u", b, counts[b], max_kp);
        most = std::max(most, counts[b]);
    }
    const size_t N = (size_t)n_images * max_kp;
    dev_scratch mem{ctx, "ochip_feature_lists_from_keypoints"};
    float *d_kp = (float *)mem.get(N * 24);
    unsigned long long *d_desc = (unsigned long long *)mem.get(N * 64);
    unsigned int *d_counts = (unsigned int *)mem.get((size_t)n_images * 4);
    int rc = d_kp && d_desc && d_counts ? OCHIP_OK : OCHIP_ENOMEM;
    if (rc == OCHIP_OK && N &&
        (hipMemcpyAsync(d_kp, kp6, N * 24, hipMemcpyHostToDevice, st) != hipSuccess ||
         hipMemcpyAsync(d_desc, desc, N * 64, hipMemcpyHostToDevice, st) != hipSuccess ||
         hipMemcpyAsync(d_counts, counts, (size_t)n_images * 4, hipMemcpyHostToDevice, st) != hipSuccess))
        rc = ochip_fail(ctx, OCHIP_EHIP, "feature lists: upload failed");
    if (rc == OCHIP_OK)
        rc = feature_lists_enqueue(ctx, mem, n_images, max_kp, d_kp, d_desc, d_counts, most, work_w, work_h, scale, nms_radius, out);
    (void)ochip_stream_wait(ctx, st);
    mem.release();
    return rc;
}
```

opencalibration_amd/csrc/host/capi_io.cpp:

```cpp
#include "../../../include/oc_host.h"

#include "capi_graph.hpp"
#include "graph_io.hpp"

#include <cstdlib>
#include <cstring>
#include <fstream>
#include <sstream>

using namespace opencalibration_amd;

struct och_checkpoint
{
    CheckpointData data;
};

namespace
{
void adopt_graph(och_graph *g, MeasurementGraph &&graph)
{
    g->graph = std::move(graph);
    g->link.reset();
    g->models.clear();
    for (const auto &node : g->graph.nodes())
// ... 32 lines not shown
    return buf;
}

int och_graph_from_json(och_graph *g, const char *text, size_t len)
{
    MeasurementGraph graph;
    std::string why;
    if (!deserialize(std::string(text, len), graph, &why))
    {
        g->error = "graph.json: " + why;
        return -1;
    }
    adopt_graph(g, std::move(graph));
    return 0;
}

int och_graph_save_json(och_graph *g, const char *path)
{
    std::ofstream out(path, std::ios::binary);
    if (!out.is_open() || !serialize(g->graph, out))
    {
        g->error = std::string("cannot write ") + path;
        return -1;
    }
    return 0;
}

int och_graph_load_json(och_graph *g, const char *path)
{
    std::ifstream in(path, std::ios::binary);
    if (!in.is_open())
    {
        g->error = std::string("cannot open ") + path;
        return -1;
    }
    const std::string text((std::istreambuf_iterator<char>(in)), std::istreambuf_iterator<char>());
    return och_graph_from_json(g, text.data(), text.size());
}

void och_graph_node_table(const och_graph *g, uint64_t *ids, uint32_t *model_index, uint64_t *n_features, uint64_t *n_sparse)
{
    size_t i = 0;
    for (const auto &node : g->graph.nodes())
    {
        if (ids)
            ids[i] = node.id;
        if (model_index)
        {
            uint32_t mi = 0;
            for (size_t k = 0; k < g->models.size(); k++)
                if (g->models[k] == node.payload.model)
                    mi = (uint32_t)k;
            model_index[i] = mi;
        }
        if (n_features)
            n_features[i] = node.payload.features.size();
        if (n_sparse)
            n_sparse[i] = node.payload.num_sparse_features;
        i++;
    }
}

int och_graph_node_payload(const och_graph *g, size_t index, double *loc, float *strength, uint64_t *desc, double *position3,
                           double *orientation4)
{
    if (index >= g->graph.size_nodes())
        return -1;
    const image &img = g->graph.nodes()[index].payload;
    for (size_t i = 0; i < img.features.size(); i++)
    {
        if (loc)
            loc[2 * i] = img.features[i].location[0], loc[2 * i + 1] = img.features[i].location[1];
        if (strength)
            strength[i] = img.features[i].strength;
        if (desc)
            std::memcpy(desc + 8 * i, img.features[i].descriptor, 64);
    }
    if (position3)
        std::memcpy(position3, img.position, 24);
    if (orientation4)
        std::memcpy(orientation4, img.orientation, 32);
    return 0;
}
const char *och_graph_node_path(const och_graph *g, size_t index)
{
    return index < g->graph.size_nodes() ? g->graph.nodes()[index].payload.path.c_str() : "";
}
int och_graph_set_node_path(och_graph *g, size_t index, const char *path)
{
    if (index >= g->graph.size_nodes())
        return -1;
    g->graph.nodes()[index].payload.path = path;
    return 0;
}

size_t och_graph_num_models(const och_graph *g)
{
    return g->models.size();
}

int och_graph_get_model(const och_graph *g, uint32_t index, double *m11)
{
    if (index >= g->models.size())
        return -1;
    const CameraModel &m = *g->models[index];
    m11[0] = m.focal_length_pixels;
    m11[1] = m.principle_point[0];
    m11[2] = m.principle_point[1];
    for (int i = 0; i < 3; i++)
        m11[3 + i] = m.radial_distortion[i];
    m11[6] = m.tangential_distortion[0];
    m11[7] = m.tangential_distortion[1];
    m11[8] = (double)m.pixels_cols;
    m11[9] = (double)m.pixels_rows;
    m11[10] = (double)m.id;
    return 0;
}

int och_surface_save_ply(const och_surface *s, const char *path)
{
    std::ofstream out(path, std::ios::binary);
    return (out.is_open() && serialize(s->s.mesh, out)) ? 0 : -1;
}

int och_surface_load_ply(och_surface *s, const char *path)
{
    std::ifstream in(path, std::ios::binary);
    if (!in.is_open())
        return -1;
    MeshGraph mesh;
    if (!deserialize(in, mesh))
        return -1;
    s->s.mesh = std::move(mesh);
    return 0;
}

size_t och_surface_num_clouds(const och_surface *s)
{
    return s->s.cloud.size();
}
void och_surface_cloud_sizes(const och_surface *s, uint64_t *sizes)
{
    for (size_t i = 0; i < s->s.cloud.size(); i++)
        sizes[i] = s->s.cloud[i].size();
}
void och_surface_set_clouds(och_surface *s, size_t n_clouds, const uint64_t *sizes, const double *xyz)
{
    s->s.cloud.assign(n_clouds, point_cloud());
    size_t k = 0;
    for (size_t i = 0; i < n_clouds; i++)
        for (uint64_t j = 0; j < sizes[i]; j++, k++)
            s->s.cloud[i].push_back({xyz[3 * k], xyz[3 * k + 1], xyz[3 * k + 2]});
}

int och_checkpoint_validate(const char *dir)
{
    return validateCheckpoint(dir) ? 1 : 0;
}

int och_checkpoint_save(const char *dir, och_graph *g, const och_surface *const *surfaces, size_t n_surfaces, const char *state,
                        const double *info4)
{
    CheckpointData data;
    data.graph = g->graph;
    for (size_t i = 0; i < n_surfaces; i++)
        data.surfaces.push_back(surfaces[i]->s);
// ... 65 lines not shown
```

opencalibration_amd/csrc/host/extract_features.cpp:

```cpp
#include "../env.hpp"
#include "extract_features.hpp"
#include "extract_slots.hpp"
#include "sort_like_std.hpp"

#include <algorithm>
#include <chrono>
#include <cmath>
#include <condition_variable>
#include <cstdio>
#include <cstdlib>
#include <cstring>
#include <deque>
#include <limits>
#include <mutex>
#include <thread>

#include <emmintrin.h>
#include <omp.h>

namespace opencalibration_amd
{

namespace
{
// ... 198 lines not shown
        {
#pragma omp atomic
            g_tail_prof[i] += d[i];
        }
    }
}

void extract_tail_prepared(const uint8_t *records, const float *response, const uint32_t *slot, uint32_t num_sparse, bool conflict,
                           uint32_t n, double scale, extracted_features &out)
{
    static const bool prof = ochip_verbose("extract");
    const double tp0 = prof ? thread_cpu_now() : 0;
    double tp1 = tp0, tp2 = tp0;
    const double nms_pixel_radius = 8;
    out.features.clear();
    out.num_sparse_features = 0;
    if (n == 0)
        return;
    const feature_2d *R = reinterpret_cast<const feature_2d *>(records);
    if (conflict)
    {
        static thread_local std::vector<by_response> recs;
        recs.resize(n);
        for (uint32_t i = 0; i < n; i++)
            recs[i] = by_response{response[i], i};
        sort_like_std(recs.data(), recs.data() + n, [](const by_response &a, const by_response &c) -> bool { return a.response > c.response; });
        if (prof)
            tp1 = thread_cpu_now();
        static thread_local std::vector<double> lx, ly;
        lx.resize(n);
        ly.resize(n);
        double minx = std::numeric_limits<double>::infinity(), miny = minx, maxx = -minx, maxy = -minx;
        for (uint32_t i = 0; i < n; i++)
        {
            const feature_2d &f = R[slot[recs[i].index]];
            lx[i] = f.location[0];
            ly[i] = f.location[1];
            minx = std::min(minx, lx[i]);
            maxx = std::max(maxx, lx[i]);
            miny = std::min(miny, ly[i]);
            maxy = std::max(maxy, ly[i]);
        }
        std::vector<uint32_t> sparse, dense;
        suppress_in_order(lx.data(), ly.data(), n, minx, miny, maxx, maxy, scale, nms_pixel_radius, sparse, dense);
        if (prof)
            tp2 = thread_cpu_now();
        out.features.reserve((size_t)n + 1);
        for (uint32_t i : sparse)
            out.features.push_back(R[slot[recs[i].index]]);
        out.num_sparse_features = out.features.size();
        for (uint32_t i : dense)
            out.features.push_back(R[slot[recs[i].index]]);
        if (prof)
        {
#pragma omp atomic
            g_tail_prof[4] += 1.0;
        }
    }
    else
    {
        out.features.assign(R, R + (size_t)n + 1);
        out.num_sparse_features = num_sparse;
    }
    if (prof)
    {
        const double tp3 = thread_cpu_now();
        const double d[4] = {tp1 - tp0, tp2 - tp1, tp3 - tp2, tp3 - tp0};
        for (int i = 0; i < 4; i++)
        {
#pragma omp atomic
            g_tail_prof[i] += d[i];
        }
    }
}

struct chunk_buffers
{
    float *kp = nullptr;
    uint64_t *desc = nullptr;
    uint8_t *prepared = nullptr;
    ochip_feature_lists lists{};
    std::vector<uint32_t> counts;
    uint32_t first = 0, n = 0;
};

extract_slots &slots_of(ochip_ctx *root)
{
    void *p = ochip_ctx_attachment(
        root, []() -> void * { return new extract_slots(); }, [](void *q) { delete static_cast<extract_slots *>(q); });
    return *static_cast<extract_slots *>(p);
}

extract_slots::order handover_order()
{
    const char *gate = std::getenv("OCHIP_EXTRACT_GATE");
    if (gate && gate[0] == '0')
        return extract_slots::order::none;
    const char *e = std::getenv("OCHIP_EXTRACT_HANDOVER");
    if (e && std::strcmp(e, "survey") == 0)
        return extract_slots::order::survey;
    return extract_slots::order::slot;
}

bool own_stream_class()
{
    const char *e = std::getenv("OCHIP_EXTRACT_PRIORITY");
    return !(e && e[0] == '0');
}

bool stagger_starts()
{
    const char *e = std::getenv("OCHIP_EXTRACT_STAGGER");
    return e && e[0] == '1';
}
}

uint32_t extract_chunk_size()
{
    if (const char *e = std::getenv("OCHIP_EXTRACT_CHUNK"))
    {
        const long v = std::atol(e);
        if (v >= 1 && v <= 1024)
            return (uint32_t)v;
    }
    return 100;
}

std::vector<extracted_features> extract_features_batch(ochip_ctx *ctx, const uint8_t *images_bgr, uint32_t n_images,
                                                       int width, int height, uint32_t max_keypoints, std::string *error,
                                                       bool images_on_device)
{
    std::vector<extracted_features> out(n_images);
    const bool ok = extract_features_stream(ctx, images_bgr, n_images, width, height, max_keypoints, images_on_device, 0,
                                            [&](uint32_t first, uint32_t count, extracted_features *f) {
                                                for (uint32_t i = 0; i < count; i++)
                                                    out[first + i] = std::move(f[i]);
                                            },
                                            error);
    if (!ok)
        return {};
    return out;
}

bool extract_features_stream(ochip_ctx *ctx, const uint8_t *images_bgr, uint32_t n_images, int width, int height,
                             uint32_t max_keypoints, bool images_on_device, int host_threads,
                             const std::function<void(uint32_t, uint32_t, extracted_features *)> &on_chunk,
                             std::string *error, extract_timing *timing)
{
    if (timing)
        *timing = extract_timing{};
    if (n_images == 0)
        return true;
    if (width <= 0 || height <= 0)
    {
        std::vector<extracted_features> empty(n_images);
        on_chunk(0, n_images, empty.data());
        return true;
    }
    const int tail_threads = host_threads > 0 ? host_threads : omp_get_max_threads();
    const int max_length_pixels = 1600;
    const double scale = std::min(1.f, float(max_length_pixels) / (float)std::max(width, height));
    const uint32_t host_chunk = 25;
    const uint32_t chunk = std::min(images_on_device ? extract_chunk_size() : host_chunk, n_images);
    const size_t image_bytes = (size_t)width * height * 3;

    uint32_t n_drivers = images_on_device ? 4 : 5;
    if (const char *e = std::getenv("OCHIP_EXTRACT_STREAMS"))
        n_drivers = (uint32_t)std::max(1L, std::min(5L, std::atol(e)));
    const uint32_t n_chunks = (n_images + chunk - 1) / chunk;
    n_drivers = std::min(n_drivers, n_chunks);
    constexpr uint32_t FIRST_SLOT_SIBLING = 21;
    const bool own_class = own_stream_class();
    std::vector<ochip_ctx *> ctxs(n_drivers, ctx);
    for (uint32_t d = own_class ? 0 : 1; d < n_drivers; d++)
        if (ochip_ctx_sibling(ctx, own_class ? FIRST_SLOT_SIBLING + d : d - 1, &ctxs[d]) != OCHIP_OK)
        {
            if (error)
                *error = std::string("ochip_ctx_sibling: ") + ochip_last_error(ctx);
            return false;
        }
    const bool device_tail = !ochip_test_hook("host_tail");
    const double nms_pixel_radius = 8;
    const bool force_host_nms = ochip_test_hook("host_nms");
    extract_slots &slots = slots_of(ctx);
    const extract_slots::order handover = handover_order();
    const auto t_enter = std::chrono::steady_clock::now();
    extract_ticket ticket(slots, n_drivers);
    constexpr int BPS = extract_slots::BUFFERS_PER_SLOT;
    const uint32_t n_bufs = BPS * n_drivers;
    std::vector<chunk_buffers> bufs(n_bufs);
    std::string fail;
    const size_t rows = (size_t)chunk * max_keypoints;
    const size_t o_resp = (rows + chunk) * 88, o_slot = o_resp + rows * 4, o_ns = o_slot + rows * 4, o_conf = o_ns + (size_t)chunk * 4;
    const size_t pad = ((size_t)chunk + 15) / 16 * 16;
    const size_t o_sub = o_conf + pad, o_nsub = o_sub + (size_t)chunk * OCHIP_SUBSET_CAP * 4, o_sconf = o_nsub + (size_t)chunk * 4;
    const size_t want[2] = {device_tail ? o_sconf + pad : rows * 6 * sizeof(float), device_tail ? 0 : rows * 8 * sizeof(uint64_t)};
    auto shape_buffer = [&](ochip_ctx *dctx, extract_slots::buffer &sb, chunk_buffers &b) -> bool {
        const int layout = device_tail ? 0 : 1;
        if (sb.layout != layout || sb.bytes[0] < want[0] || sb.bytes[1] < want[1])
        {
            for (int k = 0; k < 2; k++)
            {
                if (sb.block[k])
                    ochip_host_free(dctx, sb.block[k]);
                sb.block[k] = nullptr;
                sb.bytes[k] = 0;
            }
            sb.layout = -1;
            for (int k = 0; k < 2; k++)
                if (want[k])
                {
                    if (ochip_host_alloc(dctx, want[k], &sb.block[k]) != OCHIP_OK)
                        return false;
                    sb.bytes[k] = want[k];
                }
            sb.layout = layout;
        }
        b = chunk_buffers{};
        if (device_tail)
        {
            b.prepared = (uint8_t *)sb.block[0];
            b.lists.records = b.prepared;
            b.lists.response = (float *)(b.prepared + o_resp);
            b.lists.slot = (uint32_t *)(b.prepared + o_slot);
            b.lists.num_sparse = (uint32_t *)(b.prepared + o_ns);
            b.lists.conflict = b.prepared + o_conf;
            b.lists.subset = (uint32_t *)(b.prepared + o_sub);
            b.lists.num_subset = (uint32_t *)(b.prepared + o_nsub);
            b.lists.subset_conflict = b.prepared + o_sconf;
            b.lists.subset_spacing = 40.0;
        }
        else
        {
            b.kp = (float *)sb.block[0];
            b.desc = (uint64_t *)sb.block[1];
        }
        b.counts.resize(chunk);
        return true;
    };
    double tail_cpu_seconds = 0;
    std::mutex mu;
    std::condition_variable cv;
    std::deque<int> ready;
    uint32_t next_chunk = 0, drivers_done = 0;
    bool started = false;
    std::chrono::steady_clock::time_point t_first_slot = t_enter;
    const bool stagger = stagger_starts();
    const bool trace = ochip_verbose("extract");
    std::vector<uint64_t> progress_at_start(n_drivers, 0);
    std::vector<char> in_first_phase(n_drivers, 0);

    std::vector<double> driver_cpu(n_drivers, 0.0);
    auto driver = [&](uint32_t d) {
        ochip_ctx *dctx = ctxs[d];
        const double cpu0 = thread_cpu_now();
        struct at_exit
        {
            double &out, t0;
            ~at_exit() { out = thread_cpu_now() - t0; }
        } record{driver_cpu[d], cpu0};
        {
            slot_hold hold(slots, ticket.id(), d, handover);
            if (trace)
                fprintf(stderr, "[extract] survey %llu driver %u: slot acquired\n", (unsigned long long)ticket.id(), d);
            {
                std::lock_guard<std::mutex> lk(mu);
                if (!started)
                {
                    started = true;
                    t_first_slot = std::chrono::steady_clock::now();
                }
            }
            if (own_class && ochip_ctx_set_priority(dctx, 0) != OCHIP_OK)
            {
                std::lock_guard<std::mutex> lk(mu);
                if (fail.empty())
                    fail = std::string("ochip_ctx_set_priority: ") + ochip_last_error(dctx);
                ticket.retire();
            }
            for (;;)
            {
                uint32_t c = 0;
                bool go = false;
                {
                    std::unique_lock<std::mutex> lk(mu);
                    if (stagger)
                        while (fail.empty() && next_chunk < n_chunks)
                        {
                            bool other = false;
                            for (uint32_t o = 0; o < n_drivers; o++)
                                if (o != d && in_first_phase[o])
                                {
                                    if (ochip_akaze_progress(ctxs[o]) != progress_at_start[o])
                                        in_first_phase[o] = 0;
                                    else
                                        other = true;
                                }
                            if (!other)
                                break;
                            cv.wait_for(lk, std::chrono::milliseconds(1));
                        }
                    if (fail.empty() && next_chunk < n_chunks)
                    {
                        c = next_chunk++;
                        go = true;
                        if (stagger)
                        {
                            progress_at_start[d] = ochip_akaze_progress(dctx);
                            in_first_phase[d] = 1;
                        }
                    }
                }
                if (!go)
                    break;
                if (c + 1 == n_chunks && handover == extract_slots::order::slot)
                    ticket.retire();
                if (trace)
                    fprintf(stderr, "[extract] survey %llu driver %u: chunk %u of %u\n", (unsigned long long)ticket.id(), d, c, n_chunks);
                const int sb = slots.take_buffer(d);
                const int which = BPS * (int)d + sb;
                chunk_buffers &b = bufs[which];
                int rc = OCHIP_OK;
                if (!shape_buffer(dctx, slots.at(d, sb), b))
                    rc = OCHIP_ENOMEM;
                b.first = c * chunk;
                b.n = std::min(chunk, n_images - b.first);
                int wh[2];
                const uint8_t *src = images_bgr + (size_t)b.first * image_bytes;
                if (rc != OCHIP_OK)
                    ;
                else if (device_tail)
                    rc = images_on_device ? ochip_akaze_features_dev(dctx, src, b.n, width, height, max_keypoints, nms_pixel_radius,
                                                                     b.counts.data(), &b.lists, wh)
                                          : ochip_akaze_features(dctx, src, b.n, width, height, max_keypoints, nms_pixel_radius,
                                                                 b.counts.data(), &b.lists, wh);
                else
                    rc = images_on_device ? ochip_akaze_batch_dev(dctx, src, b.n, width, height, max_keypoints, b.kp, b.desc,
                                                                  b.counts.data(), wh)
                                          : ochip_akaze_batch(dctx, src, b.n, width, height, max_keypoints, b.kp, b.desc,
                                                              b.counts.data(), wh);
                std::unique_lock<std::mutex> lk(mu);
                in_first_phase[d] = 0;
                if (rc != OCHIP_OK)
                {
                    if (fail.empty())
                        fail = std::string("ochip_akaze_batch: ") + ochip_last_error(dctx);
                    if (trace)
                        fprintf(stderr, "[extract] survey %llu driver %u: chunk %u failed (%s)\n", (unsigned long long)ticket.id(), d, c,
                                ochip_last_error(dctx));
                    lk.unlock();
                    cv.notify_all();
                    slots.return_buffer(d, sb);
                    ticket.retire();
                    break;
                }
                ready.push_back(which);
                cv.notify_all();
            }
        }
        if (trace)
            fprintf(stderr, "[extract] survey %llu driver %u: slot released\n", (unsigned long long)ticket.id(), d);
        std::unique_lock<std::mutex> lk(mu);
        drivers_done++;
        cv.notify_all();
    };
    std::vector<std::thread> drivers;
    for (uint32_t d = 0; d < n_drivers; d++)
        drivers.emplace_back(driver, d);
    std::chrono::steady_clock::time_point t_last_final = t_enter;

    for (;;)
    {
        int which;
        {
            std::unique_lock<std::mutex> lk(mu);
            cv.wait(lk, [&] { return !ready.empty() || drivers_done == n_drivers; });
            if (ready.empty())
                break;
            which = ready.front();
            ready.pop_front();
        }
        chunk_buffers &b = bufs[which];
        double cpu = 0;
        std::vector<extracted_features> done(b.n);
#pragma omp parallel for schedule(dynamic, 1) reduction(+ : cpu) num_threads(tail_threads)
        for (uint32_t i = 0; i < b.n; i++)
        {
            const double t0 = omp_get_wtime();
            if (device_tail)
            {
                const bool conflict = b.lists.conflict[i] != 0 || force_host_nms;
                extract_tail_prepared(b.lists.records + (size_t)i * ((size_t)max_keypoints + 1) * 88,
                                      b.lists.response + (size_t)i * max_keypoints, b.lists.slot + (size_t)i * max_keypoints,
                                      b.lists.num_sparse[i], conflict, b.counts[i], scale, done[i]);
                if (!conflict && !b.lists.subset_conflict[i] && b.lists.num_subset[i] <= OCHIP_SUBSET_CAP)
                {
                    const uint32_t *sub = b.lists.subset + (size_t)i * OCHIP_SUBSET_CAP;
                    done[i].coarse_subset.assign(sub, sub + b.lists.num_subset[i]);
                    done[i].coarse_spacing = b.lists.subset_spacing;
                }
            }
            else
                extract_tail(b.kp + (size_t)i * max_keypoints * 6, b.desc + (size_t)i * max_keypoints * 8, b.counts[i], scale,
                             done[i]);
            cpu += omp_get_wtime() - t0;
        }
        tail_cpu_seconds += cpu;
        const uint32_t chunk_first = b.first, chunk_n = b.n;
        slots.return_buffer((uint32_t)(which / BPS), which % BPS);
        t_last_final = std::chrono::steady_clock::now();
        on_chunk(chunk_first, chunk_n, done.data());
    }
    for (auto &t : drivers)
        t.join();
    ticket.retire();
    if (timing)
    {
        timing->wait_seconds = std::chrono::duration<double>(t_first_slot - t_enter).count();
        timing->extract_seconds = std::chrono::duration<double>(std::max(t_last_final, t_first_slot) - t_first_slot).count();
    }
    if (ochip_verbose("extract"))
    {
        fprintf(stderr, "[extract] %u images: host tail %.3f thread-seconds of wall time (%.2f ms per image)\n", n_images,
                tail_cpu_seconds, 1e3 * tail_cpu_seconds / n_images);
        double dc = 0;
        for (double v : driver_cpu)
            dc += v;
        fprintf(stderr, "[extract] CPU seconds of the %u device driver threads (launching and waiting): %.3f\n", n_drivers, dc);
        fprintf(stderr, "[extract] cumulative CPU seconds of the tail: ordering %.3f, NMS %.3f, feature records %.3f, total %.3f; images with tied responses %.0f\n",
                g_tail_prof[0], g_tail_prof[1], g_tail_prof[2], g_tail_prof[3], g_tail_prof[4]);
    }
    if (!fail.empty())
    {
        if (error)
            *error = fail;
        return false;
    }
    return true;
}

}

extern "C" void och_extract_tail_profile(double *out5)
{
    for (int i = 0; i < 5; i++)
        out5[i] = opencalibration_amd::g_tail_prof[i];
}

extern "C" void och_sort_by_response(const float *response, uint32_t n, uint32_t *order_out, int use_std)
{
    using opencalibration_amd::by_response;
    std::vector<by_response> recs(n);
    for (uint32_t i = 0; i < n; i++)
        recs[i] = by_response{response[i], i};
    auto comp = [](const by_response &a, const by_response &c) -> bool { return a.response > c.response; };
    if (use_std)
        std::sort(recs.begin(), recs.end(), comp);
    else
        opencalibration_amd::sort_like_std(recs.data(), recs.data() + n, comp);
    for (uint32_t i = 0; i < n; i++)
        order_out[i] = recs[i].index;
}

extern "C" size_t och_extract_tail(const float *kp6, const uint64_t *desc, uint32_t n, double scale, double *loc, float *strength,
                                   uint64_t *desc_out, uint64_t *num_sparse)
// ... 31 lines not shown
```

opencalibration_amd/csrc/host/extract_features.hpp:

```cpp
#pragma once

#include "types.hpp"

#include "../../../include/ochip.h"

#include <functional>
#include <string>

namespace opencalibration_amd
{

struct extracted_features
{
    std::vector<feature_2d> features;
    size_t num_sparse_features = 0;
    std::vector<uint32_t> coarse_subset;
    double coarse_spacing = 0;
};

std::vector<extracted_features> extract_features_batch(ochip_ctx *ctx, const uint8_t *images_bgr, uint32_t n_images,
                                                       int width, int height, uint32_t max_keypoints, std::string *error,
                                                       bool images_on_device = false);

struct extract_timing
{
    double wait_seconds = 0, extract_seconds = 0;
};

bool extract_features_stream(ochip_ctx *ctx, const uint8_t *images_bgr, uint32_t n_images, int width, int height,
                             uint32_t max_keypoints, bool images_on_device, int host_threads,
                             const std::function<void(uint32_t, uint32_t, extracted_features *)> &on_chunk,
                             std::string *error, extract_timing *timing = nullptr);

}
```

opencalibration_amd/csrc/host/load_link.cpp:

```cpp
#include "../../../include/oc_host.h"

#include "capi_graph.hpp"
#include "extract_features.hpp"
#include "load_link.hpp"

#include <algorithm>
#include <atomic>
#include <chrono>
#include <condition_variable>
#include <cstdlib>
#include <deque>
#include <mutex>
#include <thread>

#include <omp.h>

using namespace opencalibration_amd;

namespace opencalibration_amd
{

std::vector<owned_pair> pair_owners(const std::vector<NodeLinks> &links)
{
    std::vector<owned_pair> out;
    std::unordered_map<size_t, size_t> link_of;
    for (size_t i = 0; i < links.size(); i++)
        link_of.emplace(links[i].node_id, i);
    for (size_t i = 0; i < links.size(); i++)
        for (size_t m : links[i].link_ids)
        {
            size_t owner = i;
            auto it = link_of.find(m);
            if (it != link_of.end() && it->second > i)
            {
                const auto &back = links[it->second].link_ids;
                if (std::find(back.begin(), back.end(), links[i].node_id) != back.end())
                    owner = it->second;
            }
            out.push_back(owned_pair{owner, LinkStage::link_pair(i, m)});
        }
    return out;
}

namespace
{
thread_local double g_last_gate_wait = 0;
std::mutex g_lane_mu;
std::condition_variable g_lane_cv;
bool g_lane_busy[2] = {false, false};
struct runner_lane
{
    int lane = -1;
    void acquire()
    {
        std::unique_lock<std::mutex> lk(g_lane_mu);
        g_lane_cv.wait(lk, [] { return !g_lane_busy[0] || !g_lane_busy[1]; });
        lane = g_lane_busy[0] ? 1 : 0;
        g_lane_busy[lane] = true;
    }
    ~runner_lane()
    {
        if (lane < 0)
            return;
        {
            std::lock_guard<std::mutex> lk(g_lane_mu);
            g_lane_busy[lane] = false;
        }
        g_lane_cv.notify_all();
    }
};
}

bool load_link_stream(och_graph *g, ochip_ctx *ctx, LinkStage &link, const std::vector<size_t> &ids, uint32_t first,
                      uint32_t count, const uint8_t *images_bgr, int width, int height, uint32_t max_keypoints,
                      bool images_on_device, const std::vector<owned_pair> &pairs, double *total_out, double *sparse_out,
                      double *t_extract_done)
{
    runner_lane lane_guard;
    lane_guard.acquire();
    const int lane = lane_guard.lane;
    g_last_gate_wait = 0;
    const auto &links = link.links();
    std::unordered_map<size_t, uint32_t> image_of;
    for (uint32_t b = 0; b < count; b++)
        image_of.emplace(ids[first + b], b);
    constexpr size_t range_len = 125;
    struct range
    {
        std::vector<LinkStage::link_pair> pairs;
        uint32_t waiting;
    };
    size_t owner_lo = links.size(), owner_hi = 0;
    for (const owned_pair &op : pairs)
    {
        owner_lo = std::min(owner_lo, op.owner);
        owner_hi = std::max(owner_hi, op.owner + 1);
    }
    const size_t n_ranges = pairs.empty() ? 0 : (owner_hi - owner_lo + range_len - 1) / range_len;
    std::vector<range> ranges(n_ranges);
    for (const owned_pair &op : pairs)
        ranges[(op.owner - owner_lo) / range_len].pairs.push_back(op.pair);
    std::vector<std::vector<uint32_t>> ranges_of_image(count);
    std::vector<uint32_t> ready_at_once;
    for (size_t k = 0; k < n_ranges; k++)
    {
        range &r = ranges[k];
        std::vector<uint32_t> need;
        for (const auto &lp : r.pairs)
        {
            auto a = image_of.find(links[lp.first].node_id);
            if (a != image_of.end())
                need.push_back(a->second);
            auto it = image_of.find(lp.second);
            if (it != image_of.end())
                need.push_back(it->second);
        }
        std::sort(need.begin(), need.end());
        need.erase(std::unique(need.begin(), need.end()), need.end());
        r.waiting = (uint32_t)need.size();
        for (uint32_t im : need)
            ranges_of_image[im].push_back((uint32_t)k);
        if (need.empty() && !r.pairs.empty())
            ready_at_once.push_back((uint32_t)k);
    }

    const char *renv = std::getenv("OCHIP_LINK_RUNNERS");
    const int n_runners = std::max(1, std::min(8, renv ? std::atoi(renv) : 3));
    const int team = omp_get_max_threads();
    const int tail_threads = std::max(1, team / 2), runner_threads = std::max(1, team / (2 * n_runners) + 1);
    std::mutex mu;
    std::condition_variable cv;
    std::deque<uint32_t> ready(ready_at_once.begin(), ready_at_once.end());
    bool no_more = false;
    std::vector<std::thread> runners;
    for (int r = 0; r < n_runners; r++)
    {
        ochip_ctx *rctx = nullptr;
        if (ochip_ctx_sibling(ctx, (uint32_t)((lane ? 13 : 4) + r), &rctx) != OCHIP_OK)
        {
            g->error = std::string("ochip_ctx_sibling: ") + ochip_last_error(ctx);
            {
                std::lock_guard<std::mutex> lk(mu);
                no_more = true;
                ready.clear();
            }
            cv.notify_all();
            for (auto &t : runners)
                t.join();
            return false;
        }
        runners.emplace_back([&, rctx]() {
            for (;;)
            {
                uint32_t k;
                {
                    std::unique_lock<std::mutex> lk(mu);
                    cv.wait(lk, [&] { return !ready.empty() || no_more; });
                    if (ready.empty())
                        return;
                    k = ready.front();
                    ready.pop_front();
                }
                link.run_pairs(g->graph, ranges[k].pairs, rctx, runner_threads);
            }
        });
    }

    double total = 0, sparse = 0;
    extract_timing timing;
    const bool ok = extract_features_stream(
        ctx, images_bgr, count, width, height, max_keypoints, images_on_device, tail_threads,
        [&](uint32_t chunk_first, uint32_t chunk_count, extracted_features *f) {
            std::vector<size_t> chunk_ids(chunk_count);
            for (uint32_t i = 0; i < chunk_count; i++)
            {
                image &img = g->graph.getNode(ids[first + chunk_first + i])->payload;
                total += (double)f[i].features.size();
                sparse += (double)f[i].num_sparse_features;
                img.features = std::move(f[i].features);
                img.num_sparse_features = f[i].num_sparse_features;
                img.coarse_subset = std::move(f[i].coarse_subset);
                img.coarse_spacing = f[i].coarse_spacing;
                chunk_ids[i] = ids[first + chunk_first + i];
            }
            link.prepare_images(g->graph, chunk_ids, tail_threads);
            std::lock_guard<std::mutex> lk(mu);
            for (uint32_t i = 0; i < chunk_count; i++)
                for (uint32_t k : ranges_of_image[chunk_first + i])
                    if (--ranges[k].waiting == 0)
                        ready.push_back(k);
            cv.notify_all();
        },
        &g->error, &timing);
    g_last_gate_wait = timing.wait_seconds;
    if (t_extract_done)
        *t_extract_done = timing.extract_seconds;
    {
        std::lock_guard<std::mutex> lk(mu);
        no_more = true;
        if (!ok)
            ready.clear();
    }
    cv.notify_all();
    for (auto &t : runners)
        t.join();
    if (!ok)
        return false;
    if (!link.error.empty())
    {
        g->error = link.error;
        return false;
    }
    if (total_out)
        *total_out = total;
    if (sparse_out)
        *sparse_out = sparse;
    return true;
}

std::vector<size_t> add_survey_nodes(och_graph *g, uint32_t n_images, uint32_t model, const double *positions,
                                     const double *orientations, uint64_t *node_ids_out)
{
    std::vector<size_t> ids(n_images);
    for (uint32_t b = 0; b < n_images; b++)
    {
        image img;
        img.model = g->models[model];
        for (int i = 0; i < 3; i++)
            img.position[i] = positions[3 * (size_t)b + i];
        if (orientations)
            for (int i = 0; i < 4; i++)
                img.orientation[i] = orientations[4 * (size_t)b + i];
        img.path = "image_" + std::to_string(g->graph.size_nodes());
        ids[b] = g->graph.addNode(std::move(img));
        if (node_ids_out)
            node_ids_out[b] = ids[b];
    }
    return ids;
}

}

extern "C" int och_graph_load_link_images(och_graph *g, ochip_ctx *ctx, const uint8_t *images_bgr, uint32_t n_images, int width,
                                          int height, uint32_t max_keypoints, int images_on_device, uint32_t model,
                                          const double *positions, const double *orientations, uint64_t *node_ids_out,
                                          double *totals2, double *link_timers8, double *stage_seconds2)
{
    using clk = std::chrono::steady_clock;
    auto seconds_since = [](clk::time_point t0) { return std::chrono::duration<double>(clk::now() - t0).count(); };
    if (!g || !ctx || (n_images && (!images_bgr || !positions)) || model >= g->models.size())
    {
        if (g)
            g->error = "och_graph_load_link_images: bad argument";
        return -1;
    }
    const auto t_begin = clk::now();
    const std::vector<size_t> ids = add_survey_nodes(g, n_images, model, positions, orientations, node_ids_out);
    g->link = std::make_unique<LinkStage>(ctx);
    LinkStage &link = *g->link;
    link.init(g->graph, ids);
    link.prepare_index(g->graph);
    {
        std::unordered_map<size_t, char> mine;
        for (size_t id : ids)
            mine.emplace(id, 1);
        std::vector<size_t> earlier;
        for (const auto &n : g->graph.nodes())
            if (!mine.count(n.id) && !n.payload.features.empty())
                earlier.push_back(n.id);
        if (!earlier.empty())
            link.prepare_images(g->graph, earlier, omp_get_max_threads());
    }
    double total = 0, sparse = 0, t_extract_done = 0;
    if (!load_link_stream(g, ctx, link, ids, 0, n_images, images_bgr, width, height, max_keypoints, images_on_device != 0,
                          pair_owners(link.links()), &total, &sparse, &t_extract_done))
        return -1;
    const double gate_wait = g_last_gate_wait;
    link.finalize(g->graph);
    if (totals2)
    {
        totals2[0] = total;
        totals2[1] = sparse;
    }
    if (link_timers8)
    {
        const LinkTimers &t = link.timers;
        const double v[8] = {t.link_init,  t.subsample,     t.upload,         t.match_device,
                             t.match_host, t.ransac_device, t.decompose_host, t.link_finalize};
        for (int i = 0; i < 8; i++)
            link_timers8[i] = v[i];
    }
    if (stage_seconds2)
    {
        stage_seconds2[0] = t_extract_done;
        stage_seconds2[1] = seconds_since(t_begin) - gate_wait;
    }
    return 0;
}
```

opencalibration_amd/host.py:

```python
import ctypes as C
import os

import numpy as np

from . import capi

_HERE = os.path.dirname(os.path.abspath(__file__))
LIB_PATH = os.path.join(_HERE, "liboc_host.so")

_lib = None
_u64p = np.ctypeslib.ndpointer(np.uint64, flags="C_CONTIGUOUS")
_f64p = np.ctypeslib.ndpointer(np.float64, flags="C_CONTIGUOUS")
_f32p = np.ctypeslib.ndpointer(np.float32, flags="C_CONTIGUOUS")


RELAX_EXCHANGE_FN = C.CFUNCTYPE(C.c_int, C.c_void_p, C.c_void_p, C.c_uint64, C.c_void_p, C.c_uint64, C.c_void_p, C.c_uint64)


def effective_cpus():
    n = len(os.sched_getaffinity(0))
    try:
        quota, period = open("/sys/fs/cgroup/cpu.max").read().split()[:2]
        if quota != "max":
            n = min(n, max(1, int(int(quota) / int(period))))
# ... 47 lines not shown
        L.och_graph_num_edges.restype = sz
        L.och_graph_node_ids.argtypes = [vp, _u64p]
        L.och_link_stage_run.argtypes = [vp, vp, _u64p, sz, C.c_int, _f64p]
        L.och_link_debug_count.argtypes = [vp]
        L.och_link_debug_count.restype = sz
        L.och_link_debug_pair.argtypes = [vp, sz, _u64p, _u64p, _f64p, np.ctypeslib.ndpointer(np.uint32)]
        L.och_link_debug_matches.argtypes = [vp, sz, _u64p, _u64p, _f64p, np.ctypeslib.ndpointer(np.uint8)]
        L.och_graph_edge_info.argtypes = [vp, sz, _u64p, _u64p, _f64p, _f64p]
        L.och_graph_edge_inliers.argtypes = [vp, sz, _u64p, _u64p, _u64p, _f64p]
        L.och_graph_edge_match_distances.argtypes = [vp, sz, _f64p]
        L.och_graph_edge_matches.argtypes = [vp, sz, vp, vp, C.POINTER(C.c_int)]
        L.och_graph_edge_matches.restype = None
        L.och_graph_set_orientations.argtypes = [vp, _f64p]
        u8p = np.ctypeslib.ndpointer(np.uint8, flags="C_CONTIGUOUS")
        L.och_relax_ground_plane.argtypes = [vp, sz, _f64p, _f64p, _f64p, sz, _u64p, _f64p, sz, _u64p, _u64p, _f64p, u8p,
                                             _u64p, _f64p, _u64p, vp, vp, sz, _u64p, _f64p, _f64p]
        L.och_relax_last_error.restype = C.c_char_p
        L.och_debug_relax_setup_check.argtypes = [C.c_int]
        L.och_graph_relax_ground_plane.argtypes = [vp, vp, _f64p, _f64p, _f64p]
        L.och_graph_relax_ground_plane_sharded.argtypes = [vp, vp, _f64p, _f64p, _f64p, u32, u32, vp, vp]
        L.och_surface_create.restype = vp
        L.och_surface_destroy.argtypes = [vp]
        L.och_surface_destroy.restype = None
        L.och_surface_counts.argtypes = [vp, C.POINTER(sz), C.POINTER(sz), C.POINTER(sz)]
        L.och_surface_counts.restype = None
        L.och_surface_get.argtypes = [vp, vp, vp, vp]
        L.och_surface_get.restype = None
        L.och_surface_set.argtypes = [vp, sz, _f64p, sz, _u64p, sz, _f64p]
        L.och_surface_set.restype = None
        L.och_surface_set_heights.argtypes = [vp, _f64p]
        L.och_surface_set_heights.restype = None
        L.och_rebuild_mesh.argtypes = [_f64p, sz, vp, C.c_int, vp]
        L.och_rebuild_mesh.restype = None
        L.och_relax.argtypes = [vp, sz, _f64p, _f64p, _f64p, _u64p, _f64p, sz, _u64p, _f64p, sz, _u64p, _u64p, vp, u8p, _u64p,
                                _f64p, _u64p, _u64p, vp, vp, sz, _u64p, u32, C.c_double, vp, vp, _f64p, vp]
        L.och_relax_ex.argtypes = L.och_relax.argtypes + [vp, C.c_int, vp, vp, sz, C.POINTER(sz)]
        L.och_graph_relax.argtypes = [vp, vp, _f64p, u32, C.c_double, vp, vp, _f64p]
        L.och_graph_relax_sharded.argtypes = [vp, vp, _f64p, u32, C.c_double, vp, vp, _f64p, u32, u32, vp, vp]
        i64p = np.ctypeslib.ndpointer(np.int64, flags="C_CONTIGUOUS")
        L.och_relax_stage_run.argtypes = [vp, vp, vp, sz, C.c_int, C.c_int, u32, C.c_double, sz, vp, vp, i64p, _f64p]
        L.och_relax_stage_begin.restype = vp
        L.och_relax_stage_begin.argtypes = [vp, vp, sz, C.c_int, C.c_int, u32, C.c_double, sz, vp, i64p]
        L.och_relax_stage_num_groups.argtypes = [vp]
        L.och_relax_stage_num_groups.restype = sz
        L.och_relax_stage_run_groups.argtypes = [vp, vp, u32, u32]
        L.och_relax_stage_export.argtypes = [vp, u32, u32, C.POINTER(vp), C.POINTER(u64)]
        L.och_relax_stage_import.argtypes = [vp, vp, u64]
        L.och_relax_stage_end.argtypes = [vp, vp, _f64p]
        L.och_relax_partition.restype = sz
        L.och_relax_partition.argtypes = [vp, sz, i64p, i64p]
        L.och_merge_surfaces.argtypes = [C.POINTER(vp), sz, vp]
        L.och_merge_surfaces.restype = None
        L.och_homography_decompose.argtypes = [_f64p, _f64p, sz, _f64p]
        L.och_image_to_3d.argtypes = [_f64p, sz, _f64p, _f64p]
        L.och_ransac_epipolar.restype = C.c_double
        L.och_ransac_epipolar.argtypes = [vp, C.c_int, _f64p, vp, sz, C.c_double, _f64p, u8p, np.ctypeslib.ndpointer(np.uint32)]
        L.och_extract_tail_prepared.restype = C.c_size_t
        L.och_extract_tail_prepared.argtypes = [C.c_void_p, _f32p, C.c_void_p, u32, C.c_int, u32, C.c_double, _f64p, _f32p, _u64p, _u64p]
        L.och_extract_tail.restype = C.c_size_t
        L.och_extract_tail.argtypes = [_f32p, _u64p, u32, C.c_double, _f64p, _f32p, _u64p, _u64p]
        L.och_graph_set_model.argtypes = [vp, u32, _f64p]
        L.och_graph_refit_edges.argtypes = [vp, vp]
        L.och_extract_features_batch.argtypes = [vp, vp, u32, C.c_int, C.c_int, u32, u32, vp, vp, vp, vp, vp, C.c_int]
        L.och_extract_last_error.restype = C.c_char_p
        L.och_graph_load_images.argtypes = [vp, vp, vp, u32, C.c_int, C.c_int, u32, C.c_int, u32, _f64p, _u64p, _f64p]
        L.och_graph_load_link_images.argtypes = [vp, vp, vp, u32, C.c_int, C.c_int, u32, C.c_int, u32, _f64p, vp, _u64p,
                                                 _f64p, _f64p, _f64p]
        L.och_initial_processing_create.restype = vp
        L.och_initial_processing_create.argtypes = [vp, vp]
        L.och_initial_processing_destroy.restype = None
        L.och_initial_processing_destroy.argtypes = [vp]
        L.och_initial_processing_pending.argtypes = [vp]
        L.och_initial_processing_step.argtypes = [vp, vp, u32, C.c_int, C.c_int, u32, C.c_int, u32, vp, C.c_int, vp, _f64p]
        L.och_graph_to_json.argtypes = [vp, C.POINTER(sz)]
        L.och_graph_to_json.restype = vp
        L.och_free.argtypes = [vp]
        L.och_free.restype = None
        L.och_graph_from_json.argtypes = [vp, C.c_char_p, sz]
        L.och_graph_save_json.argtypes = [vp, C.c_char_p]
        L.och_graph_load_json.argtypes = [vp, C.c_char_p]
        L.och_graph_node_table.argtypes = [vp, vp, vp, vp, vp]
        L.och_graph_node_table.restype = None
        L.och_graph_node_payload.argtypes = [vp, sz, vp, vp, vp, vp, vp]
        L.och_graph_node_path.argtypes = [vp, sz]
        L.och_graph_node_path.restype = C.c_char_p
        L.och_graph_set_node_path.argtypes = [vp, sz, C.c_char_p]
        L.och_graph_num_models.argtypes = [vp]
        L.och_graph_num_models.restype = sz
        L.och_graph_get_model.argtypes = [vp, u32, _f64p]
        L.och_surface_save_ply.argtypes = [vp, C.c_char_p]
        L.och_surface_load_ply.argtypes = [vp, C.c_char_p]
        L.och_surface_num_clouds.argtypes = [vp]
        L.och_surface_num_clouds.restype = sz
        L.och_surface_cloud_sizes.argtypes = [vp, _u64p]
        L.och_surface_cloud_sizes.restype = None
        L.och_surface_set_clouds.argtypes = [vp, sz, _u64p, _f64p]
        L.och_surface_set_clouds.restype = None
        L.och_checkpoint_validate.argtypes = [C.c_char_p]
        L.och_checkpoint_save.argtypes = [C.c_char_p, vp, C.POINTER(vp), sz, C.c_char_p, _f64p]
        L.och_checkpoint_load.argtypes = [C.c_char_p, vp]
        L.och_checkpoint_load.restype = vp
        L.och_checkpoint_destroy.argtypes = [vp]
        L.och_checkpoint_destroy.restype = None
        L.och_checkpoint_num_surfaces.argtypes = [vp]
        L.och_checkpoint_num_surfaces.restype = sz
        L.och_checkpoint_state.argtypes = [vp]
        L.och_checkpoint_state.restype = C.c_char_p
        L.och_checkpoint_info.argtypes = [vp, _f64p]
        L.och_checkpoint_info.restype = None
        L.och_checkpoint_get_surface.argtypes = [vp, sz, vp]
        L.och_densify_mesh.argtypes = [vp, vp, vp, _f64p, vp, sz]
        L.och_refine_by_point_density.argtypes = [vp, sz, C.c_double, C.c_int, C.c_double]
        L.och_refine_by_point_density.restype = sz
        L.och_refine_at_point.argtypes = [vp, C.c_double, C.c_double, C.c_int]
        L.och_refine_at_point.restype = sz
        L.och_count_points_per_triangle.argtypes = [vp, _u64p, _f64p, sz]
        L.och_count_points_per_triangle.restype = sz
        L.och_surface_locate.argtypes = [vp, _f64p, sz, _u64p]
        L.och_surface_locate.restype = None
        L.och_mesh_refinement_run.argtypes = [vp, vp, vp, C.c_int, _f64p]
        L.och_points_last_error.restype = C.c_char_p
        L.och_surface_count_points.argtypes = [vp, vp, _u64p, _f64p, sz]
        L.och_surface_count_points.restype = sz
        L.och_surface_locate_on.argtypes = [vp, vp, _f64p, sz, C.c_int, _u64p]
        L.och_point_counter_create.argtypes = [vp, _f64p, sz, C.c_int]
        L.och_point_counter_create.restype = vp
        L.och_point_counter_destroy.argtypes = [vp]
        L.och_point_counter_destroy.restype = None
        L.och_point_counter_count.argtypes = [vp, vp, _u64p, _f64p, sz, _u64p]
        L.och_point_counter_count.restype = sz
        L.och_surface_locate_table_sizes.argtypes = [vp, _u64p]
        L.och_surface_locate_table_sizes.restype = None
        L.och_surface_locate_table.argtypes = [vp] + [vp] * 8
        L.och_surface_locate_table.restype = None
        L.och_dense_mesh_relax_run.argtypes = [vp, vp, vp, C.c_int, _f64p]
        L.och_shard_block.argtypes = [u32, u32, u32, C.POINTER(u32), C.POINTER(u32)]
        L.och_shard_block.restype = None
        L.och_shard_begin.restype = vp
        L.och_shard_begin.argtypes = [vp, vp, u32, u32, _f64p, vp, u32, u32, _u64p]
        L.och_shard_destroy.argtypes = [vp]
        L.och_shard_destroy.restype = None
        L.och_shard_counts.argtypes = [vp, _u64p]
        L.och_shard_counts.restype = None
        L.och_shard_load_link_local.argtypes = [vp, vp, C.c_int, C.c_int, u32, C.c_int]
        for name in ("och_shard_subsets_export", "och_shard_edges_export"):
            getattr(L, name).argtypes = [vp, C.POINTER(vp), C.POINTER(u64)]
        for name in ("och_shard_subsets_import", "och_shard_edges_import"):
            getattr(L, name).argtypes = [vp, vp, u64]
        L.och_shard_link_remote.argtypes = [vp]
        L.och_shard_finalize.argtypes = [vp, _f64p, _f64p, _f64p]
        L.och_hilbert_xy2d.argtypes = [C.c_int, C.c_int, C.c_int]
        L.och_hilbert_xy2d.restype = u32
        i32, i64, f64 = C.c_int32, C.c_int64, C.c_double
        L.och_graph_set_thumbnail.argtypes = [vp, sz, sz, sz, vp]
        L.och_ortho_bounds.argtypes = [vp, sz, _f64p]
        L.och_ortho_bounds.restype = None
        L.och_ortho_gsd.argtypes = [vp, _u64p, sz, f64, C.c_int]
        L.och_ortho_gsd.restype = f64
        L.och_ortho_context.argtypes = [vp, vp, sz, C.c_int, _f64p]
        L.och_ortho_context.restype = sz
        for fn in (L.och_ortho_clamp_resolution, L.och_ortho_clamp_megapixels):
            fn.argtypes = [u64 if fn is L.och_ortho_clamp_resolution else f64, C.POINTER(f64), C.POINTER(i32), C.POINTER(i32)]
            fn.restype = None
        L.och_ray_trace_height.argtypes = [vp, sz, f64, f64, f64]
        L.och_ray_trace_height.restype = f64
        L.och_orthomosaic_thumbnail.argtypes = [vp, vp, vp, sz, vp, _f64p, vp, vp, vp]
# ... 1244 lines not shown
            self.L.och_graph_destroy(self.h)
            self.h = None

    def to_json(self):
        n = C.c_size_t(0)
        ptr = self.L.och_graph_to_json(self.h, C.byref(n))
        if not ptr:
            raise MemoryError("serialize failed")
        try:
            return C.string_at(ptr, n.value).decode("utf-8")
        finally:
            self.L.och_free(ptr)

    def _refresh_ids(self):
        ids = np.zeros(max(self.L.och_graph_num_nodes(self.h), 1), np.uint64)
        self.L.och_graph_node_ids(self.h, ids)
        self.node_ids = [int(i) for i in ids[:self.L.och_graph_num_nodes(self.h)]]

    def from_json(self, text):
        raw = text.encode("utf-8") if isinstance(text, str) else bytes(text)
        if self.L.och_graph_from_json(self.h, raw, len(raw)) != 0:
            raise ValueError(self.L.och_last_error(self.h).decode())
        self._refresh_ids()
        return self

    def save_json(self, path):
        if self.L.och_graph_save_json(self.h, str(path).encode()) != 0:
            raise IOError(self.L.och_last_error(self.h).decode())

    def load_json(self, path):
        if self.L.och_graph_load_json(self.h, str(path).encode()) != 0:
            raise ValueError(self.L.och_last_error(self.h).decode())
        self._refresh_ids()
        return self

    def densify_mesh(self, ctx, surface, want_matches=False, match_cap=1 << 22):
        stats = np.zeros(10)
        pairs = np.zeros((match_cap if want_matches else 1, 2), np.uint64)
        rc = self.L.och_densify_mesh(self.h, ctx.h, surface.h, stats, pairs.ctypes.data if want_matches else None,
                                     match_cap if want_matches else 0)
        if rc != 0:
            raise capi.OchipError("densify failed: " + self.L.och_last_error(self.h).decode())
        names = ["images", "dense_features", "queries", "matches", "tracks", "points", "index_s", "rays_s", "device_s", "tracks_s"]
        out = dict(zip(names, stats.tolist()))
        for k in names[:6]:
            out[k] = int(out[k])
        if want_matches:
            out["match_pairs"] = pairs[:min(out["matches"], match_cap)].copy()
        return out

    def mesh_refinement(self, ctx, surface=None, max_steps=40):
        surface = Surface() if surface is None else surface
        log = np.zeros((max_steps, 8))
        n = self.L.och_mesh_refinement_run(self.h, ctx.h, surface.h, max_steps, log)
        if n < 0:
            raise capi.OchipError("mesh refinement failed: " + self.L.och_last_error(self.h).decode())
        names = ["level", "grid_fraction", "gsd", "above_threshold", "max_points", "created", "vertices", "repeat"]
        return surface, [dict(zip(names, row)) for row in log[:n].tolist()]

    def dense_mesh_relax(self, surface, ctx=None, max_steps=40):
        log = np.zeros((max(max_steps, 1), 6))
        n = self.L.och_dense_mesh_relax_run(self.h, ctx.h if ctx is not None else None, surface.h, max_steps, log)
        if n < 0:
            raise capi.OchipError("dense mesh relax failed: " + self.L.och_last_error(self.h).decode())
        names = ["run", "gsd", "reduced_gsd", "above_threshold", "created", "vertices"]
        return surface, [dict(zip(names, row)) for row in log[:n].tolist()]

    def node_table(self):
        n = self.L.och_graph_num_nodes(self.h)
        ids, mi = np.zeros(max(n, 1), np.uint64), np.zeros(max(n, 1), np.uint32)
        nf, ns = np.zeros(max(n, 1), np.uint64), np.zeros(max(n, 1), np.uint64)
        self.L.och_graph_node_table(self.h, ids.ctypes.data, mi.ctypes.data, nf.ctypes.data, ns.ctypes.data)
        return dict(id=ids[:n], model=mi[:n], features=nf[:n], sparse=ns[:n])

    def node_payload(self, index):
        n = int(self.node_table()["features"][index])
        loc, st, de = np.zeros((max(n, 1), 2)), np.zeros(max(n, 1), np.float32), np.zeros((max(n, 1), 8), np.uint64)
        pos, ori = np.zeros(3), np.zeros(4)
        self.L.och_graph_node_payload(self.h, index, loc.ctypes.data, st.ctypes.data, de.ctypes.data, pos.ctypes.data,
                                      ori.ctypes.data)
        return dict(loc=loc[:n], strength=st[:n], desc=de[:n], position=pos, orientation=ori,
                    path=self.L.och_graph_node_path(self.h, index).decode("utf-8"))

    def set_node_path(self, index, path):
        self.L.och_graph_set_node_path(self.h, index, path.encode("utf-8"))

    def models(self):
        out = np.zeros((self.L.och_graph_num_models(self.h), 11))
        for i in range(len(out)):
            self.L.och_graph_get_model(self.h, i, out[i])
        return out

    def __del__(self):
        try:
            self.close()
        except Exception:
            pass

    def add_model(self, model10):
        return self.L.och_graph_add_model(self.h, np.ascontiguousarray(model10, np.float64))

    def set_model(self, model, model10):
        if self.L.och_graph_set_model(self.h, int(model), np.ascontiguousarray(model10, np.float64)) != 0:
            raise capi.OchipError("och_graph_set_model: bad model index")

    def refit_edges(self, ctx):
        if self.L.och_graph_refit_edges(self.h, ctx.h) != 0:
            raise capi.OchipError("refit failed: " + self.L.och_last_error(self.h).decode())

    def add_image(self, loc, strength, desc, num_sparse, model, position):
        nid = self.L.och_graph_add_image(self.h, np.ascontiguousarray(loc, np.float64),
                                         np.ascontiguousarray(strength, np.float32),
                                         np.ascontiguousarray(desc, np.uint64), len(strength), int(num_sparse), model,
                                         np.ascontiguousarray(position, np.float64))
        self.node_ids.append(nid)
        return nid

    def make_thumbnails(self, images_bgr, node_ids, ctx=None, device_shape=None):
        keep, src, n, h, w, on_dev = _image_batch(images_bgr, device_shape)
        ids = np.ascontiguousarray(node_ids, np.uint64).reshape(-1)
        if len(ids) != n:
            raise ValueError("one node id per image")
        ids = ids if n else np.zeros(1, np.uint64)
        if self.L.och_graph_make_thumbnails(self.h, ctx.h if ctx is not None else None, src, n, w, h, on_dev, ids) != 0:
            raise capi.OchipError("make_thumbnails failed: " + self.L.och_last_error(self.h).decode())
        del keep

    def load_images(self, ctx, images_bgr, model, positions, max_keypoints=30000, device_shape=None, thumbnails=False):
        if device_shape is None:
            imgs = np.ascontiguousarray(images_bgr, np.uint8)
            n, h, w, _ = imgs.shape
            src, on_dev = imgs.ctypes.data, 0
        else:
            n, h, w = device_shape
            src, on_dev = int(images_bgr), 1
        ids, totals = np.zeros(max(n, 1), np.uint64), np.zeros(2)
        rc = self.L.och_graph_load_images(self.h, ctx.h, src, n, w, h, max_keypoints, on_dev, model,
                                          np.ascontiguousarray(positions, np.float64).reshape(-1, 3), ids, totals)
        if rc != 0:
            raise capi.OchipError("load_images failed: " + self.L.och_last_error(self.h).decode())
        self.node_ids += [int(i) for i in ids[:n]]
        if thumbnails:
            self.make_thumbnails(images_bgr, ids[:n], ctx, device_shape)
        return totals[0] / max(n, 1), totals[1] / max(n, 1)

    def load_link_images(self, ctx, images_bgr, model, positions, orientations=None, max_keypoints=30000, device_shape=None):
        if device_shape is None:
            imgs = np.ascontiguousarray(images_bgr, np.uint8)
            n, h, w, _ = imgs.shape
            src, on_dev = imgs.ctypes.data, 0
        else:
            n, h, w = device_shape
            src, on_dev = int(images_bgr), 1
        ids, totals, timers, stage = np.zeros(max(n, 1), np.uint64), np.zeros(2), np.zeros(8), np.zeros(2)
        ori = None if orientations is None else np.ascontiguousarray(orientations, np.float64)
        rc = self.L.och_graph_load_link_images(self.h, ctx.h, src, n, w, h, max_keypoints, on_dev, model,
                                               np.ascontiguousarray(positions, np.float64).reshape(-1, 3),
                                               None if ori is None else ori.ctypes.data, ids, totals, timers, stage)
        if rc != 0:
            raise capi.OchipError("load_link_images failed: " + self.L.och_last_error(self.h).decode())
        self.node_ids += [int(i) for i in ids[:n]]
        return totals[0] / max(n, 1), totals[1] / max(n, 1), dict(zip(LINK_TIMER_NAMES, timers.tolist())), (stage[0], stage[1])

    def initial_processing(self, ctx):
        return InitialProcessing(self, ctx)

# ... 391 lines not shown
```

Before: 4180.

## Overlap feature-list readback with next extraction and balance link ranges

Splits AKAZE feature extraction into begin/finish, so the device-to-host copy of the feature lists runs on a separate copy stream from a persistent staging buffer and is synchronized by an event later. Reworks link range planning to split ranges touching the last extraction round into multiple parts, and has runners pick the largest ready range first. The aim is to hide readback latency and cut tail imbalance in the link stage. In exchange it adds cross-stream event dependencies and a reused staging buffer whose reuse must wait on the prior copy.

```diff
diff --git a/include/oc_host.h b/include/oc_host.h
--- a/include/oc_host.h
+++ b/include/oc_host.h
@@ -69,6 +69,10 @@
                                    const double *positions, const double *orientations, uint64_t *node_ids_out,
                                    double *totals2, double *link_timers8, double *stage_seconds2);
 
+    uint32_t och_link_ranges_plan(const uint64_t *owners, const int64_t *images2, uint64_t n, uint64_t range_len,
+                                  int64_t last_round_first, uint32_t tail_parts, uint32_t *range_of_pair, uint8_t *pair_in_tail);
+    uint64_t och_link_ranges_pick(const uint32_t *ready, uint64_t n_ready, const uint64_t *pairs_of_range, uint64_t n_ranges);
+
     typedef struct och_initial_processing och_initial_processing;
     och_initial_processing *och_initial_processing_create(och_graph *g, ochip_ctx *ctx);
     void och_initial_processing_destroy(och_initial_processing *ip);
@@ -167,6 +171,7 @@
     void och_graph_node_table(const och_graph *g, uint64_t *ids, uint32_t *model_index, uint64_t *n_features, uint64_t *n_sparse);
     int och_graph_node_payload(const och_graph *g, size_t index, double *loc, float *strength, uint64_t *desc,
                                double *position3, double *orientation4);
+    int64_t och_graph_node_subset(const och_graph *g, size_t index, uint32_t *out, size_t cap, double *spacing);
     const char *och_graph_node_path(const och_graph *g, size_t index);
     int och_graph_set_node_path(och_graph *g, size_t index, const char *path);
     size_t och_graph_num_models(const och_graph *g);
diff --git a/include/ochip.h b/include/ochip.h
--- a/include/ochip.h
+++ b/include/ochip.h
@@ -91,6 +91,11 @@
                              double nms_radius, uint32_t *counts, const ochip_feature_lists *lists, int *work_wh);
     int ochip_akaze_features_dev(ochip_ctx *ctx, const uint8_t *images_bgr_dev, uint32_t n_images, int width, int height,
                                  uint32_t max_kp, double nms_radius, uint32_t *counts, const ochip_feature_lists *lists, int *work_wh);
+    typedef struct ochip_akaze_pending ochip_akaze_pending;
+    int ochip_akaze_features_begin(ochip_ctx *ctx, const uint8_t *images_bgr, int images_on_device, uint32_t n_images, int width,
+                                   int height, uint32_t max_kp, double nms_radius, uint32_t *counts,
+                                   const ochip_feature_lists *lists, int *work_wh, ochip_akaze_pending **pending);
+    int ochip_akaze_features_finish(ochip_akaze_pending *pending);
     int ochip_feature_lists_from_keypoints(ochip_ctx *ctx, const float *kp6, const uint64_t *desc, const uint32_t *counts, uint32_t n_images,
                             uint32_t max_kp, int work_w, int work_h, double scale, double nms_radius,
                             const ochip_feature_lists *out);
diff --git a/opencalibration_amd/capi.py b/opencalibration_amd/capi.py
--- a/opencalibration_amd/capi.py
+++ b/opencalibration_amd/capi.py
@@ -22,7 +22,7 @@
     "ochip_descriptors_reserve", "ochip_upload_descriptors", "ochip_descriptor_count",
     "ochip_match_batch", "ochip_match_launch", "ochip_match_fetch",
     "ochip_upload_keypoints", "ochip_ransac_homography_batch", "ochip_refit_homography_batch", "ochip_ransac_epipolar_batch",
-    "ochip_upload_batch", "ochip_host_alloc", "ochip_host_free", "ochip_akaze_batch", "ochip_akaze_batch_dev", "ochip_akaze_features", "ochip_akaze_features_dev", "ochip_feature_lists_from_keypoints",
+    "ochip_upload_batch", "ochip_host_alloc", "ochip_host_free", "ochip_akaze_batch", "ochip_akaze_batch_dev", "ochip_akaze_features", "ochip_akaze_features_dev", "ochip_akaze_features_begin", "ochip_akaze_features_finish", "ochip_feature_lists_from_keypoints",
     "ochip_synth_views_alloc", "ochip_synth_views_free", "ochip_synth_render_views", "ochip_synth_views_read",
     "ochip_relax_problem_create", "ochip_relax_problem_destroy", "ochip_relax_set_cameras_constant",
     "ochip_relax_solve", "ochip_relax_get_state", "ochip_relax_set_shard", "ochip_relax_evaluate",
diff --git a/opencalibration_amd/csrc/akaze.hip b/opencalibration_amd/csrc/akaze.hip
--- a/opencalibration_amd/csrc/akaze.hip
+++ b/opencalibration_amd/csrc/akaze.hip
@@ -2608,9 +2608,14 @@
 
 int akaze_run(ochip_ctx *ctx, const uint8_t *images_bgr, bool on_device, uint32_t n_images, int width, int height,
               uint32_t max_kp, float *kp6, uint64_t *desc, uint32_t *counts, int *work_wh,
-              const ochip_feature_lists *lists = nullptr, double nms_radius = 8.0);
-
-}
+              const ochip_feature_lists *lists = nullptr, double nms_radius = 8.0, ochip_akaze_pending **pending = nullptr);
+
+}
+
+struct ochip_akaze_pending
+{
+    hipEvent_t landed = nullptr;
+};
 
 extern "C"
 {
@@ -2632,7 +2637,9 @@
 {
     if (!lists || !lists->records || !lists->response || !lists->slot || !lists->num_sparse || !lists->conflict)
         return OCHIP_EINVAL;
-    return akaze_run(ctx, images_bgr, false, n_images, width, height, max_kp, nullptr, nullptr, counts, work_wh, lists, nms_radius);
+    ochip_akaze_pending *pending = nullptr;
+    const int rc = ochip_akaze_features_begin(ctx, images_bgr, 0, n_images, width, height, max_kp, nms_radius, counts, lists, work_wh, &pending);
+    return rc != OCHIP_OK ? rc : ochip_akaze_features_finish(pending);
 }
 
 int ochip_akaze_features_dev(ochip_ctx *ctx, const uint8_t *images_bgr_dev, uint32_t n_images, int width, int height, uint32_t max_kp,
@@ -2640,7 +2647,36 @@
 {
     if (!lists || !lists->records || !lists->response || !lists->slot || !lists->num_sparse || !lists->conflict)
         return OCHIP_EINVAL;
-    return akaze_run(ctx, images_bgr_dev, true, n_images, width, height, max_kp, nullptr, nullptr, counts, work_wh, lists, nms_radius);
+    ochip_akaze_pending *pending = nullptr;
+    const int rc = ochip_akaze_features_begin(ctx, images_bgr_dev, 1, n_images, width, height, max_kp, nms_radius, counts, lists, work_wh, &pending);
+    return rc != OCHIP_OK ? rc : ochip_akaze_features_finish(pending);
+}
+
+int ochip_akaze_features_begin(ochip_ctx *ctx, const uint8_t *images_bgr, int images_on_device, uint32_t n_images, int width, int height,
+                               uint32_t max_kp, double nms_radius, uint32_t *counts, const ochip_feature_lists *lists, int *work_wh,
+                               ochip_akaze_pending **pending)
+{
+    if (!pending)
+        return OCHIP_EINVAL;
+    *pending = nullptr;
+    if (!lists || !lists->records || !lists->response || !lists->slot || !lists->num_sparse || !lists->conflict)
+        return OCHIP_EINVAL;
+    return akaze_run(ctx, images_bgr, images_on_device != 0, n_images, width, height, max_kp, nullptr, nullptr, counts, work_wh, lists,
+                     nms_radius, pending);
+}
+
+int ochip_akaze_features_finish(ochip_akaze_pending *pending)
+{
+    if (!pending)
+        return OCHIP_OK;
+    hipError_t e = hipSuccess;
+    if (pending->landed)
+    {
+        e = hipEventSynchronize(pending->landed);
+        (void)hipEventDestroy(pending->landed);
+    }
+    delete pending;
+    return e == hipSuccess ? OCHIP_OK : OCHIP_EHIP;
 }
 
 int ochip_synth_views_alloc(ochip_ctx *ctx, uint32_t n_images, int width, int height, uint8_t **images_dev)
@@ -2918,7 +2954,7 @@
 
 int akaze_run(ochip_ctx *ctx, const uint8_t *images_bgr, bool on_device, uint32_t n_images, int width, int height,
               uint32_t max_kp, float *kp6, uint64_t *desc, uint32_t *counts, int *work_wh, const ochip_feature_lists *lists,
-              double nms_radius)
+              double nms_radius, ochip_akaze_pending **pending)
 {
     if (!ctx || !counts || (n_images && (!images_bgr || (!lists && (!kp6 || !desc)))))
         return OCHIP_EINVAL;
@@ -3529,6 +3565,7 @@
     OCHIP_HIP(ctx, hipMemcpyAsync(counts, d_counts, B * 4, hipMemcpyDeviceToHost, st));
     OCHIP_HIP(ctx, ochip_stream_wait(ctx, st));
     uint32_t most = 0;
+    hipEvent_t landed = nullptr;
     for (uint32_t b = 0; b < B && rc == OCHIP_OK; b++)
     {
         if (counts[b] > max_kp)
@@ -3539,7 +3576,8 @@
         most = std::max(most, counts[b]);
     }
     if (rc == OCHIP_OK && lists)
-        rc = ochip::feature_lists_enqueue(ctx, mem, B, max_kp, d_kpc, d_descc, d_counts, most, W, H, scale, nms_radius, lists);
+        rc = ochip::feature_lists_enqueue(ctx, mem, B, max_kp, d_kpc, d_descc, d_counts, most, W, H, scale, nms_radius, lists,
+                                          pending ? &landed : nullptr);
     else if (rc == OCHIP_OK && most > 0)
     {
         OCHIP_HIP(ctx, hipMemcpy2DAsync(kp6, (size_t)max_kp * 24, d_kpc, (size_t)max_kp * 24, (size_t)most * 24, B, hipMemcpyDeviceToHost, st));
@@ -3548,7 +3586,17 @@
     if (rc != OCHIP_OK)
         for (uint32_t b = 0; b < B; b++)
             counts[b] = 0;
+    if (pending && lists && rc == OCHIP_OK)
+    {
+        *pending = new ochip_akaze_pending{landed};
+        mem.release();
+        return rc;
+    }
     (void)ochip_stream_wait(ctx, st);
+    if (pending && ctx->copy_stream)
+        (void)hipStreamSynchronize(ctx->copy_stream);
+    if (landed)
+        (void)hipEventDestroy(landed);
     mem.release();
     return rc;
 #undef AK
diff --git a/opencalibration_amd/csrc/ctx.hip b/opencalibration_amd/csrc/ctx.hip
--- a/opencalibration_amd/csrc/ctx.hip
+++ b/opencalibration_amd/csrc/ctx.hip
@@ -295,6 +295,15 @@
         ctx->lab_table_mem->release();
         delete ctx->lab_table_mem;
     }
+    if (ctx->result_stage_mem)
+    {
+        ctx->result_stage_mem->release();
+        delete ctx->result_stage_mem;
+    }
+    if (ctx->result_tail_done)
+        (void)hipEventDestroy(ctx->result_tail_done);
+    if (ctx->result_stage_free)
+        (void)hipEventDestroy(ctx->result_stage_free);
     for (auto &b : ctx->dev_pool)
         (void)hipFree(b.first);
     for (auto &b : ctx->pinned_pool)
diff --git a/opencalibration_amd/csrc/ctx.hpp b/opencalibration_amd/csrc/ctx.hpp
--- a/opencalibration_amd/csrc/ctx.hpp
+++ b/opencalibration_amd/csrc/ctx.hpp
@@ -193,6 +193,12 @@
     ochip::akaze_tables *akaze_tabs = nullptr;
     void (*akaze_tabs_destroy)(ochip::akaze_tables *) = nullptr;
 
+    ochip::dev_blocks *result_stage_mem = nullptr;
+    unsigned char *result_stage = nullptr;
+    size_t result_stage_bytes = 0;
+    hipEvent_t result_tail_done = nullptr, result_stage_free = nullptr;
+    bool result_stage_in_flight = false;
+
     void *attachment = nullptr;
     void (*attachment_destroy)(void *) = nullptr;
 };
@@ -301,7 +307,7 @@
 
 int feature_lists_enqueue(ochip_ctx *ctx, dev_blocks &mem, uint32_t B, uint32_t max_kp, const float *d_kp6,
                           const unsigned long long *d_desc, const unsigned int *d_counts, uint32_t most, int work_w, int work_h,
-                          double scale, double nms_radius, const ochip_feature_lists *out);
+                          double scale, double nms_radius, const ochip_feature_lists *out, hipEvent_t *landed = nullptr);
 
 int std_sort_enqueue(ochip_ctx *ctx, dev_blocks &mem, unsigned long long *recs, size_t total_len, const unsigned int *seg_begin,
                      const unsigned int *seg_end, uint32_t n_segs, uint32_t max_len, unsigned char *fallback);
diff --git a/opencalibration_amd/csrc/features.hip b/opencalibration_amd/csrc/features.hip
--- a/opencalibration_amd/csrc/features.hip
+++ b/opencalibration_amd/csrc/features.hip
@@ -346,9 +346,11 @@
 
 int feature_lists_enqueue(ochip_ctx *ctx, dev_blocks &mem, uint32_t B, uint32_t max_kp, const float *d_kp6,
                           const unsigned long long *d_desc, const unsigned int *d_counts, uint32_t most, int work_w, int work_h,
-                          double scale, double nms_radius, const ochip_feature_lists *out)
+                          double scale, double nms_radius, const ochip_feature_lists *out, hipEvent_t *landed)
 {
     hipStream_t st = ctx->stream;
+    if (landed)
+        *landed = nullptr;
     if (B == 0)
         return OCHIP_OK;
     if (most == 0)
@@ -396,23 +398,66 @@
         alloc_ok = alloc_ok && M.cell_id && M.cell_start && M.cell_fill && M.items && M.item_loc && M.state;
         return M;
     };
+    hipStream_t copy_st = st;
+    size_t stage_at = 0;
+    bool stage_ok = true;
+    if (landed)
+    {
+        OCHIP_HIP(ctx, ochip_copy_stream(ctx, &copy_st));
+        if (!ctx->result_tail_done)
+            OCHIP_HIP(ctx, hipEventCreateWithFlags(&ctx->result_tail_done, hipEventDisableTiming));
+        if (!ctx->result_stage_free)
+            OCHIP_HIP(ctx, hipEventCreateWithFlags(&ctx->result_stage_free, hipEventDisableTiming));
+        const size_t S_max = ((size_t)max_kp + 63) / 64 * 64, N_max = (size_t)B * S_max;
+        auto up = [](size_t b) { return (b + 255) / 256 * 256; };
+        const size_t need = 3 * up(N_max * 4) + 2 * up((size_t)B * 4) + up((size_t)B * (S_max + 1) * 88) + 2 * up(B);
+        if (ctx->result_stage_bytes < need)
+        {
+            if (ctx->result_stage_in_flight)
+                OCHIP_HIP(ctx, hipEventSynchronize(ctx->result_stage_free));
+            ctx->result_stage_in_flight = false;
+            if (!ctx->result_stage_mem)
+                ctx->result_stage_mem = new dev_blocks(ctx, "result stage");
+            ctx->result_stage_mem->release();
+            ctx->result_stage = nullptr;
+            ctx->result_stage_bytes = 0;
+            ctx->result_stage = (unsigned char *)ctx->result_stage_mem->get(need);
+            if (!ctx->result_stage)
+                return OCHIP_ENOMEM;
+            ctx->result_stage_bytes = need;
+        }
+    }
+    auto staged = [&](size_t bytes) -> void * {
+        if (!landed)
+            return dev(bytes);
+        const size_t at = stage_at;
+        stage_at += (bytes + 255) / 256 * 256;
+        if (stage_at > ctx->result_stage_bytes)
+        {
+            stage_ok = false;
+            return nullptr;
+        }
+        return ctx->result_stage + at;
+    };
     F.n = (unsigned int *)dev((size_t)B * 4);
     F.recs = (unsigned long long *)dev(N * 8);
     F.seg_begin = (unsigned int *)dev((size_t)B * 4);
     F.seg_end = (unsigned int *)dev((size_t)B * 4);
-    F.resp = (float *)dev(N * 4);
+    F.resp = (float *)staged(N * 4);
     F.loc = (double2 *)dev(N * 16);
     F.slot_of_rank = (unsigned int *)dev(N * 4);
-    F.slot = (unsigned int *)dev(N * 4);
-    F.n_sparse = (unsigned int *)dev((size_t)B * 4);
-    F.records = (unsigned char *)dev((size_t)B * (F.S + 1) * 88);
+    F.slot = (unsigned int *)staged(N * 4);
+    F.n_sparse = (unsigned int *)staged((size_t)B * 4);
+    F.records = (unsigned char *)staged((size_t)B * (F.S + 1) * 88);
     F.sub_recs = (unsigned long long *)dev(N * 8);
     F.sub_begin = (unsigned int *)dev((size_t)B * 4);
     F.sub_end = (unsigned int *)dev((size_t)B * 4);
     F.sub_loc = (double2 *)dev(N * 16);
-    F.subset = (unsigned int *)dev(N * 4);
-    F.n_subset = (unsigned int *)dev((size_t)B * 4);
-    unsigned char *conflict = (unsigned char *)dev(B), *conflict2 = (unsigned char *)dev(B);
+    F.subset = (unsigned int *)staged(N * 4);
+    F.n_subset = (unsigned int *)staged((size_t)B * 4);
+    unsigned char *conflict = (unsigned char *)staged(B), *conflict2 = (unsigned char *)staged(B);
+    if (!stage_ok)
+        return ochip_fail(ctx, OCHIP_EINVAL, "feature lists: the result stage of %zu bytes is too small", ctx->result_stage_bytes);
     if (!F.n || !F.recs || !F.seg_begin || !F.seg_end || !F.resp || !F.loc || !F.slot_of_rank || !F.slot || !F.n_sparse || !F.records ||
         !F.sub_recs || !F.sub_begin || !F.sub_end || !F.sub_loc || !F.subset || !F.n_subset || !conflict || !conflict2)
         return OCHIP_ENOMEM;
@@ -437,6 +482,8 @@
             hipLaunchKernelGGL(nms_finish_kernel<false>, dim3(B), dim3(FIN_THREADS), (size_t)F.S, st, M, F);
         return OCHIP_OK;
     };
+    if (landed && ctx->result_stage_in_flight)
+        OCHIP_HIP(ctx, hipStreamWaitEvent(st, ctx->result_stage_free, 0));
     hipLaunchKernelGGL(feat_keys_kernel, wide, dim3(256), 0, st, F);
     {
         const int src = std_sort_enqueue(ctx, mem, F.recs, N, F.seg_begin, F.seg_end, B, most, conflict);
@@ -462,20 +509,39 @@
             return rc;
     }
     OCHIP_HIP(ctx, hipGetLastError());
+    if (landed)
+    {
+        OCHIP_HIP(ctx, hipEventRecord(ctx->result_tail_done, st));
+        OCHIP_HIP(ctx, hipStreamWaitEvent(copy_st, ctx->result_tail_done, 0));
+        ctx->result_stage_in_flight = true;
+    }
     OCHIP_HIP(ctx, hipMemcpy2DAsync(out->records, ((size_t)max_kp + 1) * 88, F.records, ((size_t)F.S + 1) * 88, ((size_t)most + 1) * 88, B,
-                                    hipMemcpyDeviceToHost, st));
-    OCHIP_HIP(ctx, hipMemcpy2DAsync(out->response, (size_t)max_kp * 4, F.resp, (size_t)F.S * 4, (size_t)most * 4, B, hipMemcpyDeviceToHost, st));
-    OCHIP_HIP(ctx, hipMemcpy2DAsync(out->slot, (size_t)max_kp * 4, F.slot, (size_t)F.S * 4, (size_t)most * 4, B, hipMemcpyDeviceToHost, st));
-    OCHIP_HIP(ctx, hipMemcpyAsync(out->num_sparse, F.n_sparse, (size_t)B * 4, hipMemcpyDeviceToHost, st));
+                                    hipMemcpyDeviceToHost, copy_st));
+    OCHIP_HIP(ctx, hipMemcpy2DAsync(out->response, (size_t)max_kp * 4, F.resp, (size_t)F.S * 4, (size_t)most * 4, B, hipMemcpyDeviceToHost, copy_st));
+    OCHIP_HIP(ctx, hipMemcpy2DAsync(out->slot, (size_t)max_kp * 4, F.slot, (size_t)F.S * 4, (size_t)most * 4, B, hipMemcpyDeviceToHost, copy_st));
+    OCHIP_HIP(ctx, hipMemcpyAsync(out->num_sparse, F.n_sparse, (size_t)B * 4, hipMemcpyDeviceToHost, copy_st));
     if (want_subset)
     {
         const size_t width = std::min<size_t>(most, OCHIP_SUBSET_CAP);
         OCHIP_HIP(ctx, hipMemcpy2DAsync(out->subset, (size_t)OCHIP_SUBSET_CAP * 4, F.subset, (size_t)F.S * 4, width * 4, B,
-                                        hipMemcpyDeviceToHost, st));
-        OCHIP_HIP(ctx, hipMemcpyAsync(out->num_subset, F.n_subset, (size_t)B * 4, hipMemcpyDeviceToHost, st));
-        OCHIP_HIP(ctx, hipMemcpyAsync(out->subset_conflict, conflict2, B, hipMemcpyDeviceToHost, st));
-    }
-    OCHIP_HIP(ctx, hipMemcpyAsync(out->conflict, conflict, B, hipMemcpyDeviceToHost, st));
+                                        hipMemcpyDeviceToHost, copy_st));
+        OCHIP_HIP(ctx, hipMemcpyAsync(out->num_subset, F.n_subset, (size_t)B * 4, hipMemcpyDeviceToHost, copy_st));
+        OCHIP_HIP(ctx, hipMemcpyAsync(out->subset_conflict, conflict2, B, hipMemcpyDeviceToHost, copy_st));
+    }
+    OCHIP_HIP(ctx, hipMemcpyAsync(out->conflict, conflict, B, hipMemcpyDeviceToHost, copy_st));
+    if (landed)
+    {
+        OCHIP_HIP(ctx, hipEventRecord(ctx->result_stage_free, copy_st));
+        hipEvent_t ev = nullptr;
+        OCHIP_HIP(ctx, hipEventCreateWithFlags(&ev, hipEventBlockingSync | hipEventDisableTiming));
+        const hipError_t e = hipEventRecord(ev, copy_st);
+        if (e != hipSuccess)
+        {
+            (void)hipEventDestroy(ev);
+            OCHIP_HIP(ctx, e);
+        }
+        *landed = ev;
+    }
     return OCHIP_OK;
 }
 
diff --git a/opencalibration_amd/csrc/host/capi_io.cpp b/opencalibration_amd/csrc/host/capi_io.cpp
--- a/opencalibration_amd/csrc/host/capi_io.cpp
+++ b/opencalibration_amd/csrc/host/capi_io.cpp
@@ -138,6 +138,17 @@
         std::memcpy(orientation4, img.orientation, 32);
     return 0;
 }
+int64_t och_graph_node_subset(const och_graph *g, size_t index, uint32_t *out, size_t cap, double *spacing)
+{
+    if (index >= g->graph.size_nodes())
+        return -1;
+    const image &img = g->graph.nodes()[index].payload;
+    if (spacing)
+        *spacing = img.coarse_spacing;
+    for (size_t i = 0; out && i < img.coarse_subset.size() && i < cap; i++)
+        out[i] = (uint32_t)img.coarse_subset[i];
+    return (int64_t)img.coarse_subset.size();
+}
 const char *och_graph_node_path(const och_graph *g, size_t index)
 {
     return index < g->graph.size_nodes() ? g->graph.nodes()[index].payload.path.c_str() : "";
diff --git a/opencalibration_amd/csrc/host/extract_features.cpp b/opencalibration_amd/csrc/host/extract_features.cpp
--- a/opencalibration_amd/csrc/host/extract_features.cpp
+++ b/opencalibration_amd/csrc/host/extract_features.cpp
@@ -304,6 +304,7 @@
     ochip_feature_lists lists{};
     std::vector<uint32_t> counts;
     uint32_t first = 0, n = 0;
+    ochip_akaze_pending *pending = nullptr;
 };
 
 extract_slots &slots_of(ochip_ctx *root)
@@ -330,6 +331,12 @@
     return !(e && e[0] == '0');
 }
 
+bool overlap_results()
+{
+    const char *e = std::getenv("OCHIP_EXTRACT_OVERLAP_RESULTS");
+    return !(e && e[0] == '0');
+}
+
 bool stagger_starts()
 {
     const char *e = std::getenv("OCHIP_EXTRACT_STAGGER");
@@ -346,6 +353,21 @@
             return (uint32_t)v;
     }
     return 100;
+}
+
+extract_plan extract_plan_for(uint32_t n_images, bool images_on_device)
+{
+    extract_plan p;
+    if (n_images == 0)
+        return p;
+    const uint32_t host_chunk = 25;
+    p.chunk = std::min(images_on_device ? extract_chunk_size() : host_chunk, n_images);
+    p.n_drivers = images_on_device ? 4 : 5;
+    if (const char *e = std::getenv("OCHIP_EXTRACT_STREAMS"))
+        p.n_drivers = (uint32_t)std::max(1L, std::min(5L, std::atol(e)));
+    p.n_chunks = (n_images + p.chunk - 1) / p.chunk;
+    p.n_drivers = std::min(p.n_drivers, p.n_chunks);
+    return p;
 }
 
 std::vector<extracted_features> extract_features_batch(ochip_ctx *ctx, const uint8_t *images_bgr, uint32_t n_images,
@@ -382,15 +404,10 @@
     const int tail_threads = host_threads > 0 ? host_threads : omp_get_max_threads();
     const int max_length_pixels = 1600;
     const double scale = std::min(1.f, float(max_length_pixels) / (float)std::max(width, height));
-    const uint32_t host_chunk = 25;
-    const uint32_t chunk = std::min(images_on_device ? extract_chunk_size() : host_chunk, n_images);
+    const extract_plan plan = extract_plan_for(n_images, images_on_device);
+    const uint32_t chunk = plan.chunk, n_chunks = plan.n_chunks, n_drivers = plan.n_drivers;
     const size_t image_bytes = (size_t)width * height * 3;
 
-    uint32_t n_drivers = images_on_device ? 4 : 5;
-    if (const char *e = std::getenv("OCHIP_EXTRACT_STREAMS"))
-        n_drivers = (uint32_t)std::max(1L, std::min(5L, std::atol(e)));
-    const uint32_t n_chunks = (n_images + chunk - 1) / chunk;
-    n_drivers = std::min(n_drivers, n_chunks);
     constexpr uint32_t FIRST_SLOT_SIBLING = 21;
     const bool own_class = own_stream_class();
     std::vector<ochip_ctx *> ctxs(n_drivers, ctx);
@@ -468,6 +485,8 @@
     bool started = false;
     std::chrono::steady_clock::time_point t_first_slot = t_enter;
     const bool stagger = stagger_starts();
+    const bool overlap = overlap_results();
+    const int slow_tail_ms = ochip_test_hook("slow_tail") ? 40 : 0;
     const bool trace = ochip_verbose("extract");
     std::vector<uint64_t> progress_at_start(n_drivers, 0);
     std::vector<char> in_first_phase(n_drivers, 0);
@@ -543,6 +562,7 @@
                 const int which = BPS * (int)d + sb;
                 chunk_buffers &b = bufs[which];
                 int rc = OCHIP_OK;
+                bool finish_failed = false;
                 if (!shape_buffer(dctx, slots.at(d, sb), b))
                     rc = OCHIP_ENOMEM;
                 b.first = c * chunk;
@@ -552,10 +572,20 @@
                 if (rc != OCHIP_OK)
                     ;
                 else if (device_tail)
-                    rc = images_on_device ? ochip_akaze_features_dev(dctx, src, b.n, width, height, max_keypoints, nms_pixel_radius,
-                                                                     b.counts.data(), &b.lists, wh)
-                                          : ochip_akaze_features(dctx, src, b.n, width, height, max_keypoints, nms_pixel_radius,
-                                                                 b.counts.data(), &b.lists, wh);
+                {
+                    rc = ochip_akaze_features_begin(dctx, src, images_on_device ? 1 : 0, b.n, width, height, max_keypoints,
+                                                    nms_pixel_radius, b.counts.data(), &b.lists, wh, &b.pending);
+                    if (rc == OCHIP_OK && !overlap)
+                    {
+                        ochip_akaze_pending *p = b.pending;
+                        b.pending = nullptr;
+                        if (ochip_akaze_features_finish(p) != OCHIP_OK)
+                        {
+                            rc = OCHIP_EHIP;
+                            finish_failed = true;
+                        }
+                    }
+                }
                 else
                     rc = images_on_device ? ochip_akaze_batch_dev(dctx, src, b.n, width, height, max_keypoints, b.kp, b.desc,
                                                                   b.counts.data(), wh)
@@ -566,7 +596,8 @@
                 if (rc != OCHIP_OK)
                 {
                     if (fail.empty())
-                        fail = std::string("ochip_akaze_batch: ") + ochip_last_error(dctx);
+                        fail = finish_failed ? std::string("ochip_akaze_features_finish: the chunk's results did not arrive")
+                                             : std::string("ochip_akaze_batch: ") + ochip_last_error(dctx);
                     if (trace)
                         fprintf(stderr, "[extract] survey %llu driver %u: chunk %u failed (%s)\n", (unsigned long long)ticket.id(), d, c,
                                 ochip_last_error(dctx));
@@ -603,6 +634,24 @@
             ready.pop_front();
         }
         chunk_buffers &b = bufs[which];
+        if (b.pending)
+        {
+            ochip_akaze_pending *p = b.pending;
+            b.pending = nullptr;
+            if (ochip_akaze_features_finish(p) != OCHIP_OK)
+            {
+                {
+                    std::lock_guard<std::mutex> lk(mu);
+                    if (fail.empty())
+                        fail = "ochip_akaze_features_finish: the chunk's results did not arrive";
+                }
+                ticket.retire();
+                slots.return_buffer((uint32_t)(which / BPS), which % BPS);
+                continue;
+            }
+        }
+        if (slow_tail_ms)
+            std::this_thread::sleep_for(std::chrono::milliseconds(slow_tail_ms));
         double cpu = 0;
         std::vector<extracted_features> done(b.n);
 #pragma omp parallel for schedule(dynamic, 1) reduction(+ : cpu) num_threads(tail_threads)
diff --git a/opencalibration_amd/csrc/host/extract_features.hpp b/opencalibration_amd/csrc/host/extract_features.hpp
--- a/opencalibration_amd/csrc/host/extract_features.hpp
+++ b/opencalibration_amd/csrc/host/extract_features.hpp
@@ -27,6 +27,12 @@
     double wait_seconds = 0, extract_seconds = 0;
 };
 
+struct extract_plan
+{
+    uint32_t chunk = 0, n_chunks = 0, n_drivers = 0;
+};
+extract_plan extract_plan_for(uint32_t n_images, bool images_on_device);
+
 bool extract_features_stream(ochip_ctx *ctx, const uint8_t *images_bgr, uint32_t n_images, int width, int height,
                              uint32_t max_keypoints, bool images_on_device, int host_threads,
                              const std::function<void(uint32_t, uint32_t, extracted_features *)> &on_chunk,
diff --git a/opencalibration_amd/csrc/host/link_ranges.hpp b/opencalibration_amd/csrc/host/link_ranges.hpp
--- /dev/null
+++ b/opencalibration_amd/csrc/host/link_ranges.hpp
@@ -0,0 +1,112 @@
+#pragma once
+
+#include <algorithm>
+#include <cstddef>
+#include <cstdint>
+#include <cstdlib>
+#include <vector>
+
+namespace opencalibration_amd
+{
+
+struct planned_pair
+{
+    size_t owner;
+    int64_t image[2];
+};
+
+struct link_range_plan
+{
+    std::vector<uint32_t> range_of_pair;
+    uint32_t n_ranges = 0;
+    std::vector<uint8_t> is_tail;
+};
+
+inline size_t link_range_len()
+{
+    if (const char *e = std::getenv("OCHIP_LINK_RANGE"))
+    {
+        const long v = std::atol(e);
+        if (v >= 1 && v <= 1000000)
+            return (size_t)v;
+    }
+    return 125;
+}
+
+inline uint32_t link_tail_parts(uint32_t n_runners)
+{
+    if (const char *e = std::getenv("OCHIP_LINK_TAIL_SPLIT"))
+    {
+        const long v = std::atol(e);
+        if (v <= 0)
+            return 1;
+        if (v >= 2)
+            return (uint32_t)std::min(v, 64L);
+    }
+    return std::max(1u, n_runners);
+}
+
+inline link_range_plan plan_link_ranges(const std::vector<planned_pair> &pairs, size_t range_len, int64_t last_round_first,
+                                        uint32_t tail_parts)
+{
+    link_range_plan plan;
+    plan.range_of_pair.resize(pairs.size());
+    if (pairs.empty())
+        return plan;
+    range_len = std::max<size_t>(range_len, 1);
+    size_t owner_lo = pairs[0].owner, owner_hi = pairs[0].owner + 1;
+    for (const planned_pair &p : pairs)
+    {
+        owner_lo = std::min(owner_lo, p.owner);
+        owner_hi = std::max(owner_hi, p.owner + 1);
+    }
+    const size_t n_base = (owner_hi - owner_lo + range_len - 1) / range_len;
+    std::vector<uint8_t> base_tail(n_base, 0);
+    if (tail_parts > 1)
+        for (const planned_pair &p : pairs)
+            if (p.image[0] >= last_round_first || p.image[1] >= last_round_first)
+                base_tail[(p.owner - owner_lo) / range_len] = 1;
+    std::vector<uint32_t> first_of_base(n_base + 1, 0);
+    auto parts_of = [&](size_t b) -> size_t {
+        if (!base_tail[b])
+            return 1;
+        const size_t len = std::min(range_len, owner_hi - owner_lo - b * range_len);
+        return std::min<size_t>(tail_parts, len);
+    };
+    for (size_t b = 0; b < n_base; b++)
+        first_of_base[b + 1] = first_of_base[b] + (uint32_t)parts_of(b);
+    plan.n_ranges = first_of_base[n_base];
+    plan.is_tail.assign(plan.n_ranges, 0);
+    for (size_t b = 0; b < n_base; b++)
+        if (base_tail[b])
+            for (uint32_t k = first_of_base[b]; k < first_of_base[b + 1]; k++)
+                plan.is_tail[k] = 1;
+    for (size_t i = 0; i < pairs.size(); i++)
+    {
+        const size_t b = (pairs[i].owner - owner_lo) / range_len;
+        const size_t parts = parts_of(b);
+        uint32_t k = first_of_base[b];
+        if (parts > 1)
+        {
+            const size_t len = std::min(range_len, owner_hi - owner_lo - b * range_len);
+            const size_t at = pairs[i].owner - owner_lo - b * range_len;
+            k += (uint32_t)(at * parts / len);
+        }
+        plan.range_of_pair[i] = k;
+    }
+    return plan;
+}
+
+inline size_t pick_ready_range(const std::vector<uint32_t> &ready, const std::vector<size_t> &pairs_of_range)
+{
+    size_t best = 0;
+    for (size_t i = 1; i < ready.size(); i++)
+    {
+        const size_t a = pairs_of_range[ready[i]], b = pairs_of_range[ready[best]];
+        if (a > b || (a == b && ready[i] < ready[best]))
+            best = i;
+    }
+    return best;
+}
+
+}
diff --git a/opencalibration_amd/csrc/host/load_link.cpp b/opencalibration_amd/csrc/host/load_link.cpp
--- a/opencalibration_amd/csrc/host/load_link.cpp
+++ b/opencalibration_amd/csrc/host/load_link.cpp
@@ -2,6 +2,7 @@
 
 #include "capi_graph.hpp"
 #include "extract_features.hpp"
+#include "link_ranges.hpp"
 #include "load_link.hpp"
 
 #include <algorithm>
@@ -84,22 +85,29 @@
     std::unordered_map<size_t, uint32_t> image_of;
     for (uint32_t b = 0; b < count; b++)
         image_of.emplace(ids[first + b], b);
-    constexpr size_t range_len = 125;
     struct range
     {
         std::vector<LinkStage::link_pair> pairs;
         uint32_t waiting;
     };
-    size_t owner_lo = links.size(), owner_hi = 0;
-    for (const owned_pair &op : pairs)
-    {
-        owner_lo = std::min(owner_lo, op.owner);
-        owner_hi = std::max(owner_hi, op.owner + 1);
-    }
-    const size_t n_ranges = pairs.empty() ? 0 : (owner_hi - owner_lo + range_len - 1) / range_len;
+    const char *renv = std::getenv("OCHIP_LINK_RUNNERS");
+    const int n_runners = std::max(1, std::min(8, renv ? std::atoi(renv) : 3));
+    const extract_plan eplan = extract_plan_for(count, images_on_device);
+    const int64_t last_round_first = (int64_t)eplan.chunk * (eplan.n_chunks - eplan.n_drivers);
+    std::vector<planned_pair> planned(pairs.size());
+    for (size_t i = 0; i < pairs.size(); i++)
+    {
+        const auto a = image_of.find(links[pairs[i].pair.first].node_id), b = image_of.find(pairs[i].pair.second);
+        planned[i] = planned_pair{pairs[i].owner, {a != image_of.end() ? (int64_t)a->second : -1, b != image_of.end() ? (int64_t)b->second : -1}};
+    }
+    const link_range_plan rplan = plan_link_ranges(planned, link_range_len(), last_round_first, link_tail_parts((uint32_t)n_runners));
+    const size_t n_ranges = rplan.n_ranges;
     std::vector<range> ranges(n_ranges);
-    for (const owned_pair &op : pairs)
-        ranges[(op.owner - owner_lo) / range_len].pairs.push_back(op.pair);
+    for (size_t i = 0; i < pairs.size(); i++)
+        ranges[rplan.range_of_pair[i]].pairs.push_back(pairs[i].pair);
+    std::vector<size_t> pairs_of_range(n_ranges);
+    for (size_t k = 0; k < n_ranges; k++)
+        pairs_of_range[k] = ranges[k].pairs.size();
     std::vector<std::vector<uint32_t>> ranges_of_image(count);
     std::vector<uint32_t> ready_at_once;
     for (size_t k = 0; k < n_ranges; k++)
@@ -124,13 +132,11 @@
             ready_at_once.push_back((uint32_t)k);
     }
 
-    const char *renv = std::getenv("OCHIP_LINK_RUNNERS");
-    const int n_runners = std::max(1, std::min(8, renv ? std::atoi(renv) : 3));
     const int team = omp_get_max_threads();
     const int tail_threads = std::max(1, team / 2), runner_threads = std::max(1, team / (2 * n_runners) + 1);
     std::mutex mu;
     std::condition_variable cv;
-    std::deque<uint32_t> ready(ready_at_once.begin(), ready_at_once.end());
+    std::vector<uint32_t> ready(ready_at_once.begin(), ready_at_once.end());
     bool no_more = false;
     std::vector<std::thread> runners;
     for (int r = 0; r < n_runners; r++)
@@ -158,8 +164,9 @@
                     cv.wait(lk, [&] { return !ready.empty() || no_more; });
                     if (ready.empty())
                         return;
-                    k = ready.front();
-                    ready.pop_front();
+                    const size_t at = pick_ready_range(ready, pairs_of_range);
+                    k = ready[at];
+                    ready.erase(ready.begin() + (std::ptrdiff_t)at);
                 }
                 link.run_pairs(g->graph, ranges[k].pairs, rctx, runner_threads);
             }
@@ -241,6 +248,29 @@
 
 }
 
+extern "C" uint32_t och_link_ranges_plan(const uint64_t *owners, const int64_t *images2, uint64_t n, uint64_t range_len,
+                                         int64_t last_round_first, uint32_t tail_parts, uint32_t *range_of_pair, uint8_t *pair_in_tail)
+{
+    std::vector<planned_pair> pairs(n);
+    for (uint64_t i = 0; i < n; i++)
+        pairs[i] = planned_pair{(size_t)owners[i], {images2[2 * i], images2[2 * i + 1]}};
+    const link_range_plan plan = plan_link_ranges(pairs, (size_t)range_len, last_round_first, tail_parts);
+    for (uint64_t i = 0; i < n; i++)
+    {
+        range_of_pair[i] = plan.range_of_pair[i];
+        if (pair_in_tail)
+            pair_in_tail[i] = plan.is_tail[plan.range_of_pair[i]];
+    }
+    return plan.n_ranges;
+}
+
+extern "C" uint64_t och_link_ranges_pick(const uint32_t *ready, uint64_t n_ready, const uint64_t *pairs_of_range, uint64_t n_ranges)
+{
+    const std::vector<uint32_t> r(ready, ready + n_ready);
+    const std::vector<size_t> sizes(pairs_of_range, pairs_of_range + n_ranges);
+    return pick_ready_range(r, sizes);
+}
+
 extern "C" int och_graph_load_link_images(och_graph *g, ochip_ctx *ctx, const uint8_t *images_bgr, uint32_t n_images, int width,
                                           int height, uint32_t max_keypoints, int images_on_device, uint32_t model,
                                           const double *positions, const double *orientations, uint64_t *node_ids_out,
diff --git a/opencalibration_amd/host.py b/opencalibration_amd/host.py
--- a/opencalibration_amd/host.py
+++ b/opencalibration_amd/host.py
@@ -153,6 +153,8 @@
         L.och_graph_node_table.argtypes = [vp, vp, vp, vp, vp]
         L.och_graph_node_table.restype = None
         L.och_graph_node_payload.argtypes = [vp, sz, vp, vp, vp, vp, vp]
+        L.och_graph_node_subset.argtypes = [vp, sz, vp, sz, vp]
+        L.och_graph_node_subset.restype = C.c_int64
         L.och_graph_node_path.argtypes = [vp, sz]
         L.och_graph_node_path.restype = C.c_char_p
         L.och_graph_set_node_path.argtypes = [vp, sz, C.c_char_p]
@@ -1563,6 +1565,12 @@
         return dict(loc=loc[:n], strength=st[:n], desc=de[:n], position=pos, orientation=ori,
                     path=self.L.och_graph_node_path(self.h, index).decode("utf-8"))
 
+    def node_subset(self, index):
+        n = int(self.L.och_graph_node_subset(self.h, index, None, 0, None))
+        out, spacing = np.zeros(max(n, 1), np.uint32), C.c_double(0.0)
+        self.L.och_graph_node_subset(self.h, index, out.ctypes.data, n, C.byref(spacing))
+        return out[:n], spacing.value
+
     def set_node_path(self, index, path):
         self.L.och_graph_set_node_path(self.h, index, path.encode("utf-8"))
 
```

Result: slower. 4125 (-1.3%).
